# Clemapfel/kmer_index

Hardware: AMD Instinct MI355X
Metric: M queries/sec, DNA4 k=10 exact-match batch search, 1e8-bp text (higher is better)
Workload: dtype u32/u64

## Files before the change

include/kmx.h:

```cpp
#ifndef KMX_H
#define KMX_H

#include <stddef.h>
#include <stdint.h>

#ifdef __cplusplus
extern "C" {
#endif

#define KMX_VERSION 5
#define KMX_MAX_KS 32
#define KMX_MAX_DEVICES 16
#define KMX_QUERY_SIZE_RANGE 10000
#define KMX_SUBK_FANOUT_LIMIT 10000000ull

typedef enum kmx_status {
    KMX_OK = 0,
    KMX_ERR_INVALID_ARGUMENT = 1,
    KMX_ERR_HIP = 2,
    KMX_ERR_OUT_OF_MEMORY = 3,
    KMX_ERR_NO_DEVICE = 4,
    KMX_ERR_TOO_LARGE = 5
} kmx_status;

// ... 86 lines not shown
                                  const uint32_t** d_positions, const uint8_t** d_status);
kmx_status kmx_result_view(kmx_result* r, const uint64_t** hit_off, const uint32_t** positions,
                           const uint8_t** status, const uint8_t** kinds);

kmx_status kmx_result_parts(const kmx_result* r, uint32_t* n_parts);
kmx_status kmx_result_part_view_device(const kmx_result* r, uint32_t part, int32_t* device, uint64_t* q_begin, uint64_t* q_end,
                                       const uint64_t** d_hit_off, const uint32_t** d_positions, const uint8_t** d_status);
kmx_status kmx_index_devices(const kmx_index* index, uint32_t* n_devices, int32_t* devices);

kmx_status kmx_result_gather_device(kmx_result* r, int32_t dst_device, const uint64_t** d_hit_off, const uint32_t** d_positions,
                                    const uint8_t** d_status);

kmx_status kmx_result_masks(kmx_result* r, const uint64_t** mask_base, const uint64_t** mask_words,
                            const uint32_t** cand_count, const uint64_t** cand_src);
kmx_status kmx_index_arena_host(const kmx_index* index, const uint32_t** arena, uint64_t* n_elems);

kmx_status kmx_index_bucket_host(const kmx_index* index, uint32_t k, const uint8_t* ranks, const uint32_t** positions,
                                 uint32_t* count);

kmx_status kmx_index_levels(const kmx_index* index, uint32_t* levels);

#define KMX_PATH_INFO 1
typedef struct kmx_index_path_info {
    uint32_t struct_size;
    uint32_t fill_slots;
    uint32_t fill_nontemporal;
    uint32_t rec64;
    uint32_t tiny_cells;
    uint32_t scan_tile;
    uint32_t n_ks;
    uint32_t cell_shift[KMX_MAX_KS];
    uint32_t windows_tile;
} kmx_index_path_info;
kmx_status kmx_index_paths(const kmx_index* index, kmx_index_path_info* out);

typedef struct kmx_result_path_info {
    uint32_t struct_size;
    uint32_t small;
    uint32_t lookup_items;
    uint32_t lookup_pairs;
    uint32_t deferred_long;
    uint32_t tile_q_source;
    uint32_t spec_fill;
    uint32_t spec_ok;
    uint32_t fill_blocks;
    uint32_t fill_tiles;
    uint32_t prefix_plain;
    uint32_t prefix_small;
    uint32_t prefix_merge_small;
    uint32_t prefix_mid;
    uint32_t prefix_long;
    uint32_t prefix_large_chunks;
    uint64_t prefix_large_elems;
} kmx_result_path_info;
#define KMX_TILE_Q_NONE 0u
#define KMX_TILE_Q_PARTITION 1u
#define KMX_TILE_Q_SCAN 2u
kmx_status kmx_result_paths(const kmx_result* r, kmx_result_path_info* out);

void kmx_result_free(kmx_result* r);

#define KMX_APPROX_MAX_SUBST 3
#define KMX_APPROX_EDIT 1u
typedef struct kmx_approx_result kmx_approx_result;
kmx_status kmx_search_approx(const kmx_index* index, const uint8_t* qranks, const uint64_t* qoff, uint64_t nq,
                             uint32_t max_subst, uint32_t flags, kmx_approx_result** out);
kmx_status kmx_approx_counts(const kmx_approx_result* r, uint64_t* nq, uint64_t* n_hits, uint64_t* n_candidates,
                             uint32_t* n_chunks);
kmx_status kmx_approx_view(kmx_approx_result* r, const uint64_t** hit_off, const uint32_t** positions,
                           const uint8_t** mismatches, const uint8_t** status);
kmx_status kmx_approx_lengths(kmx_approx_result* r, const uint32_t** lengths);
void kmx_approx_free(kmx_approx_result* r);

#define KMX_APPROX_BOTH_STRANDS 1
kmx_status kmx_search_approx_strands(const kmx_index* index, const uint8_t* qranks, const uint64_t* qoff, uint64_t nq,
                                     uint32_t max_subst, uint32_t flags, const uint8_t* complement,
                                     kmx_approx_result** out);
kmx_status kmx_approx_strands(kmx_approx_result* r, const uint8_t** strands);

#define KMX_APPROX_REPORT 1
#define KMX_APPROX_LOCI 2u
#define KMX_APPROX_BEST 4u
typedef struct kmx_approx_options {
    uint32_t struct_size;
    uint32_t max_subst;
    uint32_t flags;
    uint32_t max_hits;
    const uint8_t* complement;
} kmx_approx_options;
kmx_status kmx_search_approx_opts(const kmx_index* index, const uint8_t* qranks, const uint64_t* qoff, uint64_t nq,
                                  const kmx_approx_options* options, kmx_approx_result** out);
kmx_status kmx_approx_found(kmx_approx_result* r, const uint64_t** found );

#define KMX_SEARCH_WINDOWS 1
typedef struct kmx_window_options {
    uint32_t struct_size;
    uint32_t w;
    uint32_t stride;
    uint32_t flags;
} kmx_window_options;
kmx_status kmx_search_windows(const kmx_index* index, const uint8_t* ranks, const uint64_t* roff, uint64_t nr,
                              const kmx_window_options* options, kmx_result** out);
kmx_status kmx_search_windows_device(const kmx_index* index, const void* d_ranks, const void* d_roff, uint64_t nr,
                                     const kmx_window_options* options, void* stream, kmx_result** inout);
kmx_status kmx_result_window_offsets(kmx_result* r, const uint64_t** win_off, const uint64_t** d_win_off, uint64_t* nr);

// ... 359 lines not shown
```

kmer_index_amd/build.py:

```python
import os
import shutil
import subprocess

HERE = os.path.dirname(os.path.abspath(__file__))
CSRC = os.path.join(HERE, "csrc")
LIB = os.path.join(HERE, "libkmx.so")
SOURCES = ["kmx_kernels.hip", "kmx_capi.hip", "kmx_build_sort.hip", "kmx_approx.hip", "kmx_vote.hip", "kmx_align.hip", "kmx_script.hip", "kmx_strands.hip", "kmx_pairs.hip", "kmx_rescue.hip", "kmx_tags.hip", "kmx_contigs.hip", "kmx_secondary.hip", "kmx_clip.hip", "kmx_supplementary.hip", "kmx_realign.hip", "kmx_pileup.hip", "kmx_host.cpp"]
HEADERS = ["kmx_types.h", "kmx_host.h", "kmx_kernels.h", "kmx_approx.h", "kmx_handle.h", "kmx_vote.h", "kmx_strands.h", "kmx_clips.h", "kmx_align_core.h", "kmx_script_core.h", "kmx_runs.h", "kmx_fold_core.h", os.path.join("..", "..", "include", "kmx.h")]


def _stale() -> bool:
    if not os.path.exists(LIB):
        return True
    t = os.path.getmtime(LIB)
    return any(os.path.getmtime(os.path.join(CSRC, f)) > t for f in SOURCES + HEADERS)


def build(force: bool = False, fill_e: int | None = None, verbose: bool = False, checked: bool = False) -> str:
    if not force and not _stale():
        return LIB
    hipcc = shutil.which("hipcc") or "/opt/rocm/bin/hipcc"
    cmd = [hipcc, "--offload-arch=gfx950", "-O3", "-std=c++17", "-fPIC", "-shared", "-pthread",
           "-Wall", "-Wno-unused-result", "-x", "hip"]
    if fill_e:
        cmd.append(f"-DKMX_FILL_E={fill_e}")
    for knob in ("KMX_PSORT_MULTIWAY_RUNS", "KMX_LOOKUP_OCC", "KMX_PSB_CPT", "KMX_PMERGE_MIN_AVG", "KMX_PMERGE_REG_RUNS", "KMX_PMERGE_REG_LEN", "KMX_PSORT_BAND_MIN", "KMX_SPLIT_TILE", "KMX_SPLIT_SCATTER_THREADS", "KMX_SPLIT", "KMX_NT_QUAD_LOADS", "KMX_PLAIN_QUAD_STORES", "KMX_VWAVE_OCC", "KMX_BAND", "KMX_MID_THREADS", "KMX_MID_OCC"):
        if os.environ.get(knob):
            cmd.append(f"-D{knob}={int(os.environ[knob])}")
    if os.environ.get("KMX_PHASE_TIMING"):
        cmd.append("-DKMX_PHASE_TIMING=1")
    if checked or os.environ.get("KMX_CHECKED"):
        cmd.append("-DKMX_CHECKED=1")
    cmd += [os.path.join(CSRC, f) for f in SOURCES] + ["-o", LIB]
    res = subprocess.run(cmd, capture_output=True, text=True)
    if res.returncode != 0:
        raise RuntimeError("hipcc failed:\n" + res.stdout + res.stderr)
    if verbose and (res.stdout or res.stderr):
        print(res.stdout + res.stderr)
    return LIB


if __name__ == "__main__":
    print(build(force=True, verbose=True))
```

kmer_index_amd/csrc/kmx_capi.hip:

```cpp
#include <hip/hip_runtime.h>

#include <algorithm>
#include <atomic>
#include <cstddef>
#include <cstdio>
#include <cstdlib>
#include <cstring>
#include <functional>
#include <memory>
#include <mutex>
#include <string>
#include <system_error>
#include <thread>
#include <utility>
#include <vector>

#include "kmx_approx.h"
#include "kmx_host.h"
#include "kmx_kernels.h"
#include "kmx_vote.h"

namespace {

thread_local std::string g_err;

kmx_status fail(kmx_status st, const std::string& msg)
{
    g_err = msg;
    return st;
}

#define HIP_TRY(expr)                                                                          \
    do {                                                                                       \
        hipError_t e__ = (expr);                                                               \
        if (e__ != hipSuccess) {                                                               \
            kmx_status st__ = (e__ == hipErrorOutOfMemory) ? KMX_ERR_OUT_OF_MEMORY : KMX_ERR_HIP; \
            if (e__ == hipErrorNoDevice || e__ == hipErrorInvalidDevice) st__ = KMX_ERR_NO_DEVICE; \
            return fail(st__, std::string(#expr) + ": " + hipGetErrorString(e__));             \
        }                                                                                      \
    } while (0)

#define KMX_TRY(expr) do { const kmx_status try_st__ = (expr); if (try_st__ != KMX_OK) return try_st__; } while (0)
struct DevBuf {
    void* p = nullptr;
    size_t cap = 0;
    hipError_t ensure(size_t bytes)
    {
        if (bytes <= cap) return hipSuccess;
        if (p) { (void)hipFree(p); p = nullptr; cap = 0; }
        size_t want = bytes + bytes / 16 + 256;
        hipError_t e = hipMalloc(&p, want);
        if (e != hipSuccess) { p = nullptr; return e; }
        cap = want;
        return hipSuccess;
    }
    void release()
    {
        if (p) (void)hipFree(p);
        p = nullptr; cap = 0;
    }
    template <typename T> T* as() const { return static_cast<T*>(p); }
};

struct HostBuf {
    void* p = nullptr;
    size_t cap = 0;
    bool pinned = false;
    bool ensure(size_t bytes)
    {
        if (bytes <= cap) return true;
        release();
// ... 62 lines not shown
    void drain()
    {
        for (auto& p : pending) {
            (void)hipEventSynchronize(p.b);
            float t = 0.f;
            if (hipEventElapsedTime(&t, p.a, p.b) == hipSuccess) { ms[p.id] += t; launches[p.id] += 1; }
            pool.push_back(p.a);
            pool.push_back(p.b);
        }
        pending.clear();
    }
    void destroy()
    {
        drain();
        for (auto e : pool) (void)hipEventDestroy(e);
        pool.clear();
    }
};

}

struct ResultPool {
    std::mutex mu;
    std::vector<kmx_result*> idle;
    std::vector<kmx_result*> pending;
    bool closed = false;
};
constexpr size_t kPoolMaxResults = 8;
constexpr size_t kPoolMaxBytes = size_t(256) << 20;
constexpr size_t kSmallView = size_t(256) << 10;

struct kmx_index {
    std::shared_ptr<ResultPool> pool = std::make_shared<ResultPool>();
    int device = 0;
    uint64_t n = 0;
    uint32_t sigma = 0;
    uint32_t range = KMX_QUERY_SIZE_RANGE;
    std::vector<uint32_t> ks;
    std::vector<uint32_t> table_kinds;
    std::vector<void*> allocs;
    uint64_t device_bytes = 0;
    uint64_t bytes_positions = 0, bytes_aligned = 0, bytes_cells = 0, bytes_levels = 0;
    KmxIndexDev* d_index = nullptr;
    KmxIndexDev* d_index_fast = nullptr;
    const KmxPlanEntry* d_plan_fast = nullptr;
    const uint32_t* d_arena = nullptr;
    unsigned long long* d_dbg = nullptr;
    struct ElemSizes { size_t n_offs, n_slots, n_ukeys, n_aoffs; };
    std::vector<ElemSizes> elem_sizes;
    std::vector<uint8_t> tail;
    KmxIndexDev h_header{};
    kmx::FillVariant fill_variant{12, true};
    bool rec32 = true;
    bool tiny_cells = false;
    bool broken = false;
    std::vector<uint32_t> host_arena;
    Stats stats;
    struct HostDir {
        std::once_flag once;
        kmx_status st = KMX_OK;
        std::string err;
        std::vector<uint32_t> offs;
        std::vector<uint64_t> ukeys;
    };
    std::unique_ptr<HostDir[]> host_dirs;
    std::vector<kmx_index*> peers;
    std::unique_ptr<kmx::PackedText> text = std::make_unique<kmx::PackedText>();
    kmx::ContigTable contigs;
    std::vector<uint64_t> h_contigs;
    size_t n_replicas() const { return 1 + peers.size(); }
    kmx_index* replica(size_t i) { return i ? peers[i - 1] : this; }
};

struct SearchCtx {
    kmx_index* ix = nullptr;
    const uint8_t* qr = nullptr;
    const uint64_t* qo = nullptr;
    hipStream_t s = nullptr;
    uint64_t tile_cap = 0, spec_tiles = 0;
    bool spec_fill = false;
    bool pending = false;
};

struct Tallies {
    uint64_t n_hits = 0, n_exact = 0, n_stitch = 0, n_prefix = 0, n_error = 0, n_none = 0, n_mask_words = 0;
    void reset() { *this = Tallies{}; }
    void operator+=(const Tallies& o) { n_hits += o.n_hits; n_exact += o.n_exact; n_stitch += o.n_stitch; n_prefix += o.n_prefix; n_error += o.n_error; n_none += o.n_none; n_mask_words += o.n_mask_words; }
    void derive_exact(uint64_t nq) { n_exact = nq - n_stitch - n_prefix - n_error - n_none; }
};
constexpr size_t kCtrBytes = KMX_CTR_COUNT * sizeof(unsigned long long);

struct kmx_result : Tallies {
    const kmx_index* index = nullptr;
    int device = 0;
    hipStream_t stream = nullptr;
    uint32_t flags = 0;
    uint64_t nq = 0;
    DevBuf src, cnt, c0, aux, key, p1, kind, status, stitch_list, prefix_list, short_list, hit_off, bsum, ctr, tile_q, out,
        mask_words, stitch_hits, plen, poff, ptmp, pitems, pbands, pcuts, pbanded, psplits, ptiles, pscnt, pscratch, pmid, in_qranks, in_qoff, win_cnt, win_off;
    unsigned long long* h_ctr = nullptr;
    HostBuf h_hit_off, h_positions, h_status, h_kinds, h_mask_base, h_mask_words, h_cand_count, h_cand_src, h_small;
    uint64_t* v_hit_off = nullptr; uint32_t* v_positions = nullptr; uint8_t* v_status = nullptr; uint8_t* v_kinds = nullptr;
    const uint64_t* m_base = nullptr; const uint64_t* m_words = nullptr; const uint32_t* m_ccnt = nullptr; const uint64_t* m_csrc = nullptr;
    uint32_t ctr_phase = 0;
    bool ctr_clean = false;
    HostBuf mailbox, small_in;
    DevBuf small_xchg;
    bool small_valid = false;
    bool host_valid = false, host_masks_valid = false;
    bool windows = false, h_win_valid = false;
    uint64_t win_nr = 0, win_n = 0;
    uint32_t win_w = 0, win_stride = 0;
    HostBuf h_win_off;
    bool last_had_stitch = false;
    bool last_had_long = false;
    bool last_had_pairs = false;
    struct PathRec { uint32_t small = 0, items = 0, pairs = 0, defer_long = 0, tile_q_source = 0, spec_fill = 0, spec_ok = 0, fill_blocks = 0, fill_tiles = 0;
                     uint32_t p_plain = 0, p_small = 0, p_merge = 0, p_mid = 0, p_long = 0, p_chunks = 0; uint64_t p_elems = 0; };
    PathRec path;
    std::shared_ptr<ResultPool> pool;
    SearchCtx ctx;
    hipEvent_t done = nullptr;
    bool quiesced = true;
    hipStream_t own_stream = nullptr;
    std::vector<kmx_result*> parts;
    std::vector<uint64_t> part_q0;
    std::vector<uint64_t> part_w0;
    bool chunked = false;
    bool host_chunk = false;
    kmx_result* worker = nullptr;
    kmx_result* worker2 = nullptr;
    DevBuf g_hit_off, g_out, g_status;
    int gather_device = -1;
    hipStream_t gather_stream = nullptr;

    Tallies& tally() { return *this; }
    template <typename R, typename F> static void each_device_buffer(R& r, F&& f)
    {
        for (auto* b : {&r.src, &r.cnt, &r.c0, &r.aux, &r.key, &r.p1, &r.kind, &r.status, &r.stitch_list, &r.prefix_list, &r.short_list, &r.hit_off, &r.bsum,
                        &r.ctr, &r.tile_q, &r.out, &r.mask_words, &r.stitch_hits, &r.plen, &r.poff, &r.ptmp, &r.pitems, &r.pbands, &r.pcuts, &r.pbanded, &r.psplits,
                        &r.ptiles, &r.pscnt, &r.pscratch, &r.pmid, &r.in_qranks, &r.in_qoff, &r.small_xchg, &r.win_cnt, &r.win_off})
            f(*b);
    }
    size_t device_bytes() const { size_t b = 0; each_device_buffer(*this, [&](const DevBuf& d) { b += d.cap; }); return b; }
    kmx::QueryDesc query_desc() const
    {
        return kmx::QueryDesc{src.as<uint64_t>(), cnt.as<uint32_t>(), c0.as<uint32_t>(), aux.as<uint64_t>(), key.as<uint64_t>(), p1.as<uint64_t>(),
                              kind.as<uint8_t>(), status.as<uint8_t>(), stitch_list.as<uint32_t>(), prefix_list.as<uint32_t>(), short_list.as<uint32_t>(), nullptr};
    }
    unsigned long long* ctr_block(uint32_t phase) const { return ctr.as<unsigned long long>() + phase * KMX_CTR_COUNT; }
    hipError_t ensure_h_ctr() { return h_ctr ? hipSuccess : hipHostMalloc(reinterpret_cast<void**>(&h_ctr), kCtrBytes, hipHostMallocDefault); }
    void view_own() { v_hit_off = h_hit_off.as<uint64_t>(); v_positions = h_positions.as<uint32_t>(); v_status = h_status.as<uint8_t>(); v_kinds = h_kinds.as<uint8_t>(); }
    void mask_view_own() { m_base = h_mask_base.as<uint64_t>(); m_words = h_mask_words.as<uint64_t>(); m_ccnt = h_cand_count.as<uint32_t>(); m_csrc = h_cand_src.as<uint64_t>(); }
    bool size_views(uint64_t pos_bytes)
    {
        const uint64_t nq1 = std::max<uint64_t>(nq, 1);
        const bool ok = h_hit_off.ensure((nq + 1) * 8) && h_status.ensure(nq1) && h_kinds.ensure(nq1) && h_positions.ensure(std::max<uint64_t>(pos_bytes, 4));
        if (ok) view_own();
        return ok;
    }
    bool size_mask_buffers()
    {
        const uint64_t nq1 = std::max<uint64_t>(nq, 1);
        return h_mask_base.ensure(nq1 * 8) && h_cand_count.ensure(nq1 * 4) && h_cand_src.ensure(nq1 * 8) &&
               h_mask_words.ensure(std::max<uint64_t>(n_mask_words, 1) * 8);
    }

    void release_gather()
    {
        (void)hipSetDevice(gather_device);
// ... 53 lines not shown
    launch();
    (void)hipEventRecord(b, s);
    ix->stats.pending.push_back({id, a, b});
}

template <typename T>
kmx_status upload(kmx_index* ix, const T* host, size_t count, const T** dev_out)
{
    void* p = nullptr;
    size_t bytes = std::max<size_t>(count * sizeof(T), 16) + 16;
    HIP_TRY(hipMalloc(&p, bytes));
    ix->allocs.push_back(p);
    ix->device_bytes += bytes;
    if (count) HIP_TRY(hipMemcpy(p, host, count * sizeof(T), hipMemcpyHostToDevice));
    *dev_out = static_cast<const T*>(p);
    return KMX_OK;
}

struct DeviceScratch {
    std::vector<void*> ptrs;
    ~DeviceScratch() { for (void* p : ptrs) (void)hipFree(p); }
    template <typename T> hipError_t get(T** out, size_t count)
    {
        void* p = nullptr;
        hipError_t e = hipMalloc(&p, count * sizeof(T) + 64);
        if (e == hipSuccess) { ptrs.push_back(p); *out = static_cast<T*>(p); }
        return e;
    }
};

kmx_status check_device()
{
    int count = 0;
    hipError_t e = hipGetDeviceCount(&count);
    if (e != hipSuccess || count <= 0)
        return fail(KMX_ERR_NO_DEVICE, "no HIP device visible: the kmx engine has no CPU search path");
    return KMX_OK;
}

}

static uint32_t cell_shift_for(uint32_t table_kind, uint64_t n_keys, uint64_t npos, uint64_t region, const kmx_options& o)
{
    if (table_kind != KMX_TABLE_DENSE || o.no_aligned_copy || region > npos) return 0;
    if (const char* e = getenv("KMX_CELLS")) { if (!atoi(e)) return 0; }
    const double c = double(npos) / double(n_keys);
    uint32_t shift = c <= 3.5 ? 3u : c <= 10.5 ? 4u : c <= 24.0 ? 5u : 0u;
    if (const char* e = getenv("KMX_CELL_SHIFT")) { const int v = atoi(e); if (v >= 3 && v <= 5) shift = uint32_t(v); }
    if (!shift) return 0;
    if ((n_keys << shift) > 8 * npos) return 0;
    return shift;
}
static inline uint64_t up32_elems(uint64_t v) { return (v + 31) & ~uint64_t(31); }

static hipError_t publish_headers(kmx_index* ix)
{
    hipError_t e = hipMemcpy(ix->d_index, &ix->h_header, sizeof(KmxIndexDev), hipMemcpyHostToDevice);
    if (e == hipSuccess && ix->d_index_fast) {
        KmxIndexDev hf = ix->h_header;
        if (ix->d_plan_fast) hf.plan = ix->d_plan_fast;
        e = hipMemcpy(ix->d_index_fast, &hf, sizeof hf, hipMemcpyHostToDevice);
    }
    return e;
}
static inline const KmxIndexDev* header_for(const kmx_index* ix, uint32_t flags)
{
    static const bool ref_plan_only = getenv("KMX_REFERENCE_PLAN") != nullptr;
    return ((flags & (KMX_SEARCH_KEEP_MASKS | KMX_SEARCH_REFERENCE_PLAN)) || !ix->d_index_fast || ref_plan_only) ? ix->d_index : ix->d_index_fast;
}

static kmx_status install_images_impl(std::vector<kmx::ElemImage>& images, const uint8_t* tail_kmax, uint64_t n, uint32_t sigma,
                                 uint32_t range, int device, const kmx_options& o, kmx_index** out, void* prebuilt_arena,
                                 uint64_t prebuilt_arena_elems = 0)
{
    auto* ix = new kmx_index();
    ix->device = device;
    ix->n = n;
    ix->sigma = sigma;
    ix->range = range;
    const uint32_t n_ks = uint32_t(images.size());
    uint32_t kmax = 0;
    for (auto& im : images) { ix->ks.push_back(im.k); kmax = std::max(kmax, im.k); }
    kmx_status st = KMX_OK;
    auto bail = [&](kmx_status s) { std::string keep = g_err; kmx_index_free(ix); g_err = keep; return s; };
    for (auto& im : images) {
        if (im.d_offs_prebuilt) ix->allocs.push_back(const_cast<uint32_t*>(im.d_offs_prebuilt));
        if (im.d_atab_prebuilt) ix->allocs.push_back(const_cast<uint32_t*>(im.d_atab_prebuilt));
        if (im.d_ukeys_prebuilt) ix->allocs.push_back(const_cast<uint64_t*>(im.d_ukeys_prebuilt));
        if (im.d_slots_prebuilt) ix->allocs.push_back(const_cast<KmxSlot*>(im.d_slots_prebuilt));
    }

    KmxIndexDev h{};
    h.n = n; h.sigma = sigma; h.n_ks = n_ks; h.kmax = kmax; h.range = range;
    for (uint32_t j = 0; j < 64; ++j) {
        unsigned __int128 v = 1;
        for (uint32_t t = 0; t < j; ++t) { v *= sigma; if (v > ~uint64_t(0)) { v = ~uint64_t(0); break; } }
        h.pw[j] = uint64_t(v);
    }
    uint64_t arena_elems = 0;
    for (auto& im : images) {
        if (!im.region) im.region = im.npos;
        if (im.region > im.npos) arena_elems = (arena_elems + 31) & ~uint64_t(31);
        arena_elems += im.region;
    }
    std::vector<uint32_t> cell_shift(n_ks, 0);
    std::vector<uint64_t> cell_base(n_ks, 0);
// ... 66 lines not shown
            ix->elem_sizes.back() = {size_t(nu + 1), size_t(cap), size_t(nu), size_t(0)};
        } else if (im.d_offs_prebuilt) {
            el.offs = im.d_offs_prebuilt;
            ix->device_bytes += (im.n_keys + 1) * 4;
            ix->elem_sizes.back().n_offs = im.n_keys + 1;
        } else if ((st = upload(ix, im.offs.data(), im.offs.size(), &el.offs)) != KMX_OK) return bail(st);
        if (im.d_atab_prebuilt) {
            el.atab = im.d_atab_prebuilt;
            ix->device_bytes += (im.n_keys + 1) * 4;
        } else if (im.table_kind == KMX_TABLE_DENSE && !im.atab.empty()) {
            if ((st = upload(ix, im.atab.data(), im.atab.size(), &el.atab)) != KMX_OK) return bail(st);
        }
        if (im.table_kind == KMX_TABLE_OPEN && !im.d_ukeys_prebuilt) {
            if ((st = upload(ix, im.slots.data(), im.slots.size(), &el.slots)) != KMX_OK) return bail(st);
            if ((st = upload(ix, im.ukeys.data(), im.ukeys.size(), &el.ukeys)) != KMX_OK) return bail(st);
        }
        el.dir = nullptr; el.dir_shift = 0; el.n_dir = 0;
        if (im.table_kind == KMX_TABLE_OPEN && el.n_ukeys >= 1024) {
            uint32_t key_bits = 1;
            while (key_bits < 64 && (im.n_keys - 1) >> key_bits) ++key_bits;
            uint32_t lg = 0;
            while ((uint64_t(1) << lg) < el.n_ukeys) ++lg;
            const uint32_t D = std::min<uint32_t>(std::min<uint32_t>(20, key_bits), lg > 8 ? lg - 4 : 4);
            void* p = nullptr;
            if (hipMalloc(&p, ((size_t(1) << D) + 1) * 4 + 64) == hipSuccess) {
                ix->allocs.push_back(p);
                ix->device_bytes += ((size_t(1) << D) + 1) * 4;
                el.dir = static_cast<const uint32_t*>(p);
                el.dir_shift = key_bits - D;
                el.n_dir = 1u << D;
                kmx::launch_build_dir(nullptr, el.ukeys, el.n_ukeys, el.dir_shift, el.n_dir, static_cast<uint32_t*>(p));
                hipError_t le = hipGetLastError();
                if (le == hipSuccess) le = hipDeviceSynchronize();
                if (le != hipSuccess) { fail(KMX_ERR_HIP, std::string("key directory: ") + hipGetErrorString(le)); return bail(KMX_ERR_HIP); }
            } else {
                (void)hipGetLastError();
            }
        }
        el.cnt8 = nullptr; el.cell_base = 0; el.cell_shift = 0; el.n_levels = 0;
        if (cell_shift[i]) {
            void* p = nullptr;
            hipError_t ce = hipMalloc(&p, im.n_keys + 64);
            if (ce == hipSuccess) {
                ix->allocs.push_back(p);
                ix->device_bytes += im.n_keys;
                (void)hipMemset(p, 0, im.n_keys + 64);
                kmx::launch_build_cells(nullptr, el.offs, h.arena + base, im.n_keys, cell_shift[i], const_cast<uint32_t*>(h.arena) + cell_base[i],
                                        static_cast<uint8_t*>(p));
                ce = hipGetLastError();
                if (ce == hipSuccess) ce = hipDeviceSynchronize();
            }
            if (ce != hipSuccess) { fail(ce == hipErrorOutOfMemory ? KMX_ERR_OUT_OF_MEMORY : KMX_ERR_HIP, std::string("cells: ") + hipGetErrorString(ce)); return bail(KMX_ERR_HIP); }
            el.cnt8 = static_cast<const uint8_t*>(p);
            if (im.npos <= 4 * im.n_keys) ix->tiny_cells = true;
            ix->bytes_cells += ((im.n_keys << cell_shift[i]) * 4) + im.n_keys;
            el.cell_base = cell_base[i];
            el.cell_shift = cell_shift[i];
            if (o.keep_host_arena) {
                ce = hipMemcpy(ix->host_arena.data() + cell_base[i], h.arena + cell_base[i], (im.n_keys << cell_shift[i]) * 4, hipMemcpyDeviceToHost);
                if (ce != hipSuccess) { fail(KMX_ERR_HIP, std::string("cells download: ") + hipGetErrorString(ce)); return bail(KMX_ERR_HIP); }
            }
        }
        base += im.region;
        im = kmx::ElemImage();
    }
    ix->host_dirs.reset(new kmx_index::HostDir[n_ks]);
    ix->tail.assign(tail_kmax, tail_kmax + kmax);
    if ((st = upload(ix, tail_kmax, kmax, &h.tail)) != KMX_OK) return bail(st);
    {
        std::vector<KmxPlanEntry> plan = kmx::make_plan_entries(ix->ks, range);
        if ((st = upload(ix, plan.data(), plan.size(), &h.plan)) != KMX_OK) return bail(st);
    }
    {
        const KmxIndexDev* d = nullptr;
        if ((st = upload(ix, &h, 1, &d)) != KMX_OK) return bail(st);
        ix->d_index = const_cast<KmxIndexDev*>(d);
        ix->h_header = h;
        std::vector<KmxPlanEntry> fast = kmx::make_fast_plan_entries(ix->ks, range, sigma);
        if ((st = upload(ix, fast.data(), fast.size(), &ix->d_plan_fast)) != KMX_OK) return bail(st);
        if ((st = upload(ix, &h, 1, &d)) != KMX_OK) return bail(st);
        ix->d_index_fast = const_cast<KmxIndexDev*>(d);
        const hipError_t pe = publish_headers(ix);
        if (pe != hipSuccess) { fail(KMX_ERR_HIP, std::string("header: ") + hipGetErrorString(pe)); return bail(KMX_ERR_HIP); }
    }
    *out = ix;
    return KMX_OK;
}

static kmx_status replicate_index(const kmx_index* src, int device, kmx_index** out)
{
    auto* ix = new kmx_index();
    ix->device = device;
    ix->n = src->n; ix->sigma = src->sigma; ix->range = src->range;
    ix->ks = src->ks; ix->table_kinds = src->table_kinds; ix->elem_sizes = src->elem_sizes; ix->tail = src->tail;
    ix->fill_variant = src->fill_variant; ix->rec32 = src->rec32; ix->tiny_cells = src->tiny_cells;
    ix->bytes_positions = src->bytes_positions; ix->bytes_aligned = src->bytes_aligned; ix->bytes_cells = src->bytes_cells; ix->bytes_levels = src->bytes_levels;
    auto bail = [&](kmx_status s) { std::string keep = g_err; kmx_index_free(ix); g_err = keep; return s; };
    hipError_t e = hipSetDevice(device);
    if (e != hipSuccess) { fail(KMX_ERR_NO_DEVICE, std::string("replica device: ") + hipGetErrorString(e)); return bail(KMX_ERR_NO_DEVICE); }
    kmx_status st = KMX_OK;
    auto clone = [&](const void* sp, size_t bytes, size_t pad, const void** dp) -> bool {
        *dp = nullptr;
        if (!sp) return true;
        void* p = nullptr;
        hipError_t e2 = hipMalloc(&p, std::max<size_t>(bytes, 16) + pad);
        if (e2 != hipSuccess) { st = fail(KMX_ERR_OUT_OF_MEMORY, std::string("replica: ") + hipGetErrorString(e2)); return false; }
        ix->allocs.push_back(p);
        ix->device_bytes += bytes;
        if (bytes) {
            e2 = hipMemcpyPeer(p, device, sp, src->device, bytes);
            if (e2 != hipSuccess) { st = fail(KMX_ERR_HIP, std::string("replica copy: ") + hipGetErrorString(e2)); return false; }
        }
        *dp = p;
        return true;
    };
    KmxIndexDev h = src->h_header;
    const void* p = nullptr;
    if (!clone(src->h_header.arena, h.arena_elems * 4 + KMX_ARENA_PAD, 0, &p)) return bail(st);
    h.arena = static_cast<const uint32_t*>(p); ix->d_arena = h.arena;
    if (!clone(src->h_header.tail, h.kmax, 16, &p)) return bail(st);
    h.tail = static_cast<const uint8_t*>(p);
    if (!clone(src->h_header.plan, size_t(h.range) * sizeof(KmxPlanEntry), 16, &p)) return bail(st);
    h.plan = static_cast<const KmxPlanEntry*>(p);
    if (!clone(src->d_plan_fast, src->d_plan_fast ? size_t(h.range) * sizeof(KmxPlanEntry) : 0, 16, &p)) return bail(st);
    ix->d_plan_fast = static_cast<const KmxPlanEntry*>(p);
    {
        void* d = nullptr;
        if (hipMalloc(&d, 16 * 8) == hipSuccess) { (void)hipMemset(d, 0, 16 * 8); ix->allocs.push_back(d); h.dbg = static_cast<unsigned long long*>(d); ix->d_dbg = h.dbg; }
        else { (void)hipGetLastError(); h.dbg = nullptr; }
    }
    for (uint32_t i = 0; i < h.n_ks; ++i) {
        const KmxElemDev& se = src->h_header.elems[i];
        KmxElemDev& de = h.elems[i];
        const auto& sz = src->elem_sizes[i];
        if (!clone(se.offs, sz.n_offs * 4, 16, &p)) return bail(st);
        de.offs = static_cast<const uint32_t*>(p);
        if (!clone(se.atab, sz.n_aoffs * 4, 16, &p)) return bail(st);
        de.atab = static_cast<const uint32_t*>(p);
        if (!clone(se.slots, sz.n_slots * sizeof(KmxSlot), 16, &p)) return bail(st);
        de.slots = static_cast<const KmxSlot*>(p);
        if (!clone(se.ukeys, sz.n_ukeys * 8, 16, &p)) return bail(st);
        de.ukeys = static_cast<const uint64_t*>(p);
        if (!clone(se.dir, se.dir ? (size_t(se.n_dir) + 1) * 4 : 0, 64, &p)) return bail(st);
        de.dir = static_cast<const uint32_t*>(p);
        if (!clone(se.cnt8, se.cnt8 ? size_t(se.n_keys) : 0, 64, &p)) return bail(st);
        de.cnt8 = static_cast<const uint8_t*>(p);
    }
    if (!clone(nullptr, 0, 0, &p)) return bail(st);
// ... 688 lines not shown
            if (he == hipSuccess && !hd.ukeys.empty()) he = hipMemcpy(hd.ukeys.data(), el.ukeys, hd.ukeys.size() * 8, hipMemcpyDeviceToHost);
            if (he != hipSuccess) { hd.st = KMX_ERR_HIP; hd.err = std::string("kmx_index_bucket_host: table download: ") + hipGetErrorString(he); }
        }
        if (have) (void)hipSetDevice(cur);
    });
    if (hd.st != KMX_OK) return fail(hd.st, hd.err);
    uint64_t g = h;
    if (el.table_kind == KMX_TABLE_OPEN) {
        const auto it = std::lower_bound(hd.ukeys.begin(), hd.ukeys.end(), h);
        if (it == hd.ukeys.end() || *it != h) return KMX_OK;
        g = uint64_t(it - hd.ukeys.begin());
    }
    if (g + 1 >= hd.offs.size()) return KMX_OK;
    const uint32_t a = hd.offs[g], b = hd.offs[g + 1];
    if (b == a) return KMX_OK;
    *positions = ix->host_arena.data() + el.arena_base + a;
    *count = b - a;
    return KMX_OK;
}

kmx_status kmx_index_levels(const kmx_index* ix, uint32_t* levels)
{
    if (!ix || !levels) return fail(KMX_ERR_INVALID_ARGUMENT, "kmx_index_levels: NULL argument");
    for (size_t i = 0; i < ix->ks.size(); ++i) levels[i] = ix->h_header.elems[i].n_levels;
    return KMX_OK;
}

kmx_status kmx_index_paths(const kmx_index* ix, kmx_index_path_info* out)
{
    if (!ix || !out || out->struct_size < sizeof(uint32_t)) return fail(KMX_ERR_INVALID_ARGUMENT, "kmx_index_paths: NULL argument or no struct_size");
    const kmx::FillVariant fv = kmx::effective_fill_variant(ix->fill_variant, ix->rec32);
    kmx_index_path_info v{};
    v.fill_slots = uint32_t(fv.e); v.fill_nontemporal = fv.nt; v.rec64 = !ix->rec32; v.tiny_cells = ix->tiny_cells;
    v.scan_tile = uint32_t(kmx::scan_tile());
    v.n_ks = uint32_t(ix->ks.size());
    for (size_t i = 0; i < ix->ks.size(); ++i) v.cell_shift[i] = ix->h_header.elems[i].cnt8 ? ix->h_header.elems[i].cell_shift : 0u;
    v.windows_tile = uint32_t(kmx::windows_tile());
    v.struct_size = std::min<uint32_t>(out->struct_size, uint32_t(sizeof v));
    memcpy(out, &v, v.struct_size);
    return KMX_OK;
}

kmx_status kmx_result_paths(const kmx_result* r, kmx_result_path_info* out)
{
    if (!r || !out || out->struct_size < sizeof(uint32_t)) return fail(KMX_ERR_INVALID_ARGUMENT, "kmx_result_paths: NULL argument or no struct_size");
    if (!r->parts.empty()) return fail(KMX_ERR_INVALID_ARGUMENT, "kmx_result_paths: a result of several parts has no single search to report");
    KMX_TRY(search_finish(const_cast<kmx_result*>(r)));
    kmx_result_path_info v{};
    v.small = r->path.small; v.lookup_items = r->path.items; v.lookup_pairs = r->path.pairs; v.deferred_long = r->path.defer_long;
    v.tile_q_source = r->path.tile_q_source; v.spec_fill = r->path.spec_fill; v.spec_ok = r->path.spec_ok;
    v.fill_blocks = r->path.fill_blocks; v.fill_tiles = r->path.fill_tiles;
    v.prefix_plain = r->path.p_plain; v.prefix_small = r->path.p_small; v.prefix_merge_small = r->path.p_merge; v.prefix_mid = r->path.p_mid;
    v.prefix_long = r->path.p_long; v.prefix_large_chunks = r->path.p_chunks; v.prefix_large_elems = r->path.p_elems;
    v.struct_size = std::min<uint32_t>(out->struct_size, uint32_t(sizeof v));
    memcpy(out, &v, v.struct_size);
    return KMX_OK;
}

kmx_status kmx_debug_words(const kmx_index* ix, uint64_t* words16)
{
    if (!ix || !words16 || !ix->d_dbg) return fail(KMX_ERR_INVALID_ARGUMENT, "kmx_debug_words: NULL argument");
    HIP_TRY(hipSetDevice(ix->device));
    HIP_TRY(hipDeviceSynchronize());
    HIP_TRY(hipMemcpy(words16, ix->d_dbg, 16 * 8, hipMemcpyDeviceToHost));
    return KMX_OK;
}

kmx_status kmx_stats_enable(kmx_index* ix, int enable)
{
    if (!ix) return fail(KMX_ERR_INVALID_ARGUMENT, "kmx_stats_enable: index is NULL");
    for (kmx_index* peer : ix->peers) (void)kmx_stats_enable(peer, enable);
    std::lock_guard<std::mutex> lock(ix->stats.mu);
    ix->stats.enabled = enable != 0;
    return KMX_OK;
}

kmx_status kmx_stats_get(kmx_index* ix, kmx_kernel_stat* stats, uint32_t* n)
{
    if (!ix || !stats || !n) return fail(KMX_ERR_INVALID_ARGUMENT, "kmx_stats_get: NULL argument");
    {
        std::lock_guard<std::mutex> lock(ix->stats.mu);
        (void)hipSetDevice(ix->device);
        ix->stats.drain();
        for (int i = 0; i < K_COUNT; ++i) stats[i] = kmx_kernel_stat{kKernelNames[i], ix->stats.launches[i], ix->stats.ms[i]};
    }
    for (kmx_index* peer : ix->peers) {
        std::lock_guard<std::mutex> lock(peer->stats.mu);
        (void)hipSetDevice(peer->device);
        peer->stats.drain();
        for (int i = 0; i < K_COUNT; ++i) { stats[i].launches += peer->stats.launches[i]; stats[i].total_ms += peer->stats.ms[i]; }
    }
    if (!ix->peers.empty()) (void)hipSetDevice(ix->device);
    *n = K_COUNT;
    return KMX_OK;
}

kmx_status kmx_stats_reset(kmx_index* ix)
{
    if (!ix) return fail(KMX_ERR_INVALID_ARGUMENT, "kmx_stats_reset: index is NULL");
    for (kmx_index* peer : ix->peers) (void)kmx_stats_reset(peer);
    std::lock_guard<std::mutex> lock(ix->stats.mu);
    (void)hipSetDevice(ix->device);
    ix->stats.drain();
    for (int i = 0; i < K_COUNT; ++i) { ix->stats.launches[i] = 0; ix->stats.ms[i] = 0; }
    return KMX_OK;
}

static kmx_status search_device_begin(const kmx_index* cix, const void* d_first, bool nonempty, kmx_result** inout, const char* fn, const char* what,
                                      kmx_index** ix_out)
{
    const std::string f = std::string(fn) + ": ";
    kmx_index* ix = const_cast<kmx_index*>(cix);
    if (ix->broken) return fail(KMX_ERR_HIP, "the index is unusable: a failed kmx_index_extend_query_size_range left its replicas inconsistent");
    if (!ix->peers.empty() && nonempty) {
        hipPointerAttribute_t attr{};
        if (hipPointerGetAttributes(&attr, d_first) != hipSuccess) { (void)hipGetLastError(); return fail(KMX_ERR_INVALID_ARGUMENT, f + what + " is not a device pointer"); }
        kmx_index* pick = nullptr;
        for (size_t i = 0; i < ix->n_replicas() && !pick; ++i)
            if (ix->replica(i)->device == attr.device) pick = ix->replica(i);
        if (!pick) return fail(KMX_ERR_INVALID_ARGUMENT, f + "the queries live on a device that holds no replica of this index");
        ix = pick;
    }
    HIP_TRY(hipSetDevice(ix->device));
    kmx_result* r = *inout;
    if (r && !r->parts.empty()) return fail(KMX_ERR_INVALID_ARGUMENT, f + "the result handle belongs to a multi-device search");
    if (r && r->device != ix->device && r->device_bytes())
        return fail(KMX_ERR_INVALID_ARGUMENT, f + "the result handle holds buffers on another device");
    if (!r) { r = take_result(ix); *inout = r; }
    else KMX_TRY(search_finish(r));
    *ix_out = ix;
    return KMX_OK;
}

static bool scan_hits(kmx_index* ix, kmx_result* r, hipStream_t s, uint64_t tile, uint64_t tile_cap, int items, const kmx::CounterPub& pub)
{
    bool published = false;
    timed(ix, K_SCAN, s, [&] {
        published = kmx::launch_scan_tiles(s, r->cnt.as<uint32_t>(), r->nq, r->bsum.as<uint64_t>(), r->hit_off.as<uint64_t>(),
                                           r->ctr_block(r->ctr_phase) + KMX_CTR_TOTAL_HITS, tile, tile_cap >= 2 ? tile_cap - 1 : 0,
                                           tile_cap >= 2 ? r->tile_q.as<uint32_t>() : nullptr, items, pub);
    });
    return published;
}

using LookupStep = std::function<int(const kmx::QueryDesc&, unsigned long long*, const KmxIndexDev*)>;
static kmx_status search_device_run(kmx_index* ix, kmx_result* r, const uint8_t* qr, const uint64_t* qo, uint64_t nq, uint32_t flags, hipStream_t s,
                                    const LookupStep& lookup)
{
    r->index = ix; r->device = ix->device; r->stream = s;
    (void)hipGetLastError();
    r->flags = flags;
    r->nq = nq;
    r->tally().reset();
    r->host_valid = r->host_masks_valid = false;
    r->small_valid = false;
    r->path = kmx_result::PathRec{};
    r->quiesced = false;
    HIP_TRY(r->ensure_h_ctr());
    HIP_TRY(r->hit_off.ensure((nq + 1) * 8));
    if (nq == 0) {
        HIP_TRY(hipMemsetAsync(r->hit_off.p, 0, 8, s));
        return KMX_OK;
    }
    const std::pair<DevBuf*, size_t> per_query[] = {{&r->src, 8}, {&r->cnt, 4}, {&r->c0, 4}, {&r->aux, 8}, {&r->key, 8}, {&r->p1, 8}, {&r->kind, 1},
                                                    {&r->status, 1}, {&r->stitch_list, 4}, {&r->prefix_list, 4}, {&r->short_list, 4}};
    for (const auto& b : per_query) HIP_TRY(b.first->ensure(nq * b.second));
    HIP_TRY(r->bsum.ensure(std::max(kmx::scan_blocks(nq), kmx::lookup_blocks(nq, 4)) * 8));
    if (r->ctr.cap < 2 * kCtrBytes) {
        HIP_TRY(r->ctr.ensure(2 * kCtrBytes));
        HIP_TRY(hipMemsetAsync(r->ctr.p, 0, 2 * kCtrBytes, s));
        r->ctr_phase = 0;
        r->ctr_clean = true;
    }
    const kmx::QueryDesc d = r->query_desc();
    if (!r->ctr_clean) {
        HIP_TRY(hipMemsetAsync(r->ctr.p, 0, 2 * kCtrBytes, s));
        r->ctr_clean = true;
    }
    r->ctr_phase ^= 1u;
    auto* ctr = r->ctr_block(r->ctr_phase);
    auto* ctr_next = r->ctr_block(r->ctr_phase ^ 1u);
    const KmxIndexDev* dix = header_for(ix, flags);

    const int items = lookup(d, ctr, dix);
    const kmx::FillVariant fv = kmx::effective_fill_variant(ix->fill_variant, ix->rec32);
    const uint64_t tile = kmx::fill_tile(fv);
    const uint64_t tile_cap = r->tile_q.cap / 4;
    const bool published = scan_hits(ix, r, s, tile, tile_cap, items, kmx::CounterPub{ctr, ctr_next, r->h_ctr});
    r->ctr_clean = published;
    const uint64_t spec_tiles = std::min<uint64_t>(tile_cap >= 2 ? tile_cap - 1 : 0, (r->out.cap / 4) / tile);
    const bool spec_fill = !(flags & KMX_SEARCH_COUNT_ONLY) && !r->last_had_stitch && spec_tiles > 0 && spec_tiles < 0x7FFFFFFFull;
    if (spec_fill)
        timed(ix, K_FILL, s, [&] {
            kmx::launch_fill(s, fv, ix->rec32, dix, ix->d_arena, r->hit_off.as<uint64_t>(), r->tile_q.as<uint32_t>(),
                             ctr + KMX_CTR_TOTAL_HITS, spec_tiles, d, r->out.as<uint32_t>());
        });
    r->path.spec_fill = spec_fill;
    if (!published) HIP_TRY(hipMemcpyAsync(r->h_ctr, ctr, kCtrBytes, hipMemcpyDeviceToHost, s));
    r->ctx = SearchCtx{ix, qr, qo, s, tile_cap, spec_tiles, spec_fill, true};
    if (flags & KMX_SEARCH_ASYNC) {
        if (!r->done) HIP_TRY(hipEventCreateWithFlags(&r->done, hipEventDisableTiming));
        HIP_TRY(hipEventRecord(r->done, s));
        r->pool = ix->pool;
        std::lock_guard<std::mutex> lock(ix->pool->mu);
        ix->pool->pending.push_back(r);
        return KMX_OK;
    }
    return search_finish(r);
}

kmx_status kmx_search_batch_device(const kmx_index* cix, const void* d_qranks, const void* d_qoff, uint64_t nq,
                                   uint32_t flags, void* stream, kmx_result** inout)
{
    if (!cix || !inout) return fail(KMX_ERR_INVALID_ARGUMENT, "kmx_search_batch_device: NULL argument");
    if (nq && (!d_qranks || !d_qoff)) return fail(KMX_ERR_INVALID_ARGUMENT, "kmx_search_batch_device: NULL query buffers");
    if (nq >= 0xFFFFFFFFull) return fail(KMX_ERR_INVALID_ARGUMENT, "kmx_search_batch_device: at most 2^32-2 queries per batch");
    kmx_index* ix = nullptr;
    KMX_TRY(search_device_begin(cix, d_qranks, nq != 0, inout, "kmx_search_batch_device", "d_qranks", &ix));
    hipStream_t s = static_cast<hipStream_t>(stream);
    const uint8_t* qr = static_cast<const uint8_t*>(d_qranks);
    const uint64_t* qo = static_cast<const uint64_t*>(d_qoff);
    kmx_result* r = *inout;
    r->windows = false;
    return search_device_run(ix, r, qr, qo, nq, flags, s, [&](const kmx::QueryDesc& d, unsigned long long* ctr, const KmxIndexDev* dix) {
        static const int force_items = getenv("KMX_LOOKUP_ITEMS") ? atoi(getenv("KMX_LOOKUP_ITEMS")) : 0;
        const bool pairs = force_items ? force_items == -4 : r->last_had_pairs;
        const int items = force_items ? (force_items == 8 ? 8 : 4) : (!pairs && ix->tiny_cells) ? 8 : 4;
        const bool defer_long = r->last_had_long;
        const uint32_t lflags = (flags & ~KMX_SEARCH_INTERNAL_DEFER_LONG) | (defer_long ? KMX_SEARCH_INTERNAL_DEFER_LONG : 0u);
        r->path.items = uint32_t(items); r->path.pairs = pairs; r->path.defer_long = defer_long;
        timed(ix, K_LOOKUP, s, [&] {
            kmx::launch_lookup(s, items, pairs, dix, qr, qo, nq, d, ctr, r->bsum.as<uint64_t>(), lflags);
            if (defer_long) kmx::launch_lookup_long(s, dix, qr, qo, nq, d, ctr, flags);
        });
        return items;
    });
}


static kmx_status windows_check(const char* fn, const kmx_index* ix, const kmx_window_options* o, const void* out, uint32_t* elem)
{
    const std::string f = std::string(fn) + ": ";
    if (!ix || !o || !out) return fail(KMX_ERR_INVALID_ARGUMENT, f + "NULL argument");
    if (o->struct_size < sizeof(kmx_window_options)) return fail(KMX_ERR_INVALID_ARGUMENT, f + "options->struct_size is too small");
    if (o->stride == 0) return fail(KMX_ERR_INVALID_ARGUMENT, f + "stride must be at least 1");
    if (o->flags & ~uint32_t(KMX_SEARCH_COUNT_ONLY))
        return fail(KMX_ERR_INVALID_ARGUMENT, f + "flags other than KMX_SEARCH_COUNT_ONLY have nothing to act on");
    for (size_t i = 0; i < ix->ks.size(); ++i)
        if (ix->ks[i] == o->w) { *elem = uint32_t(i); return KMX_OK; }
    return fail(KMX_ERR_INVALID_ARGUMENT, f + "w = " + std::to_string(o->w) + " is not the k of an element of the index");
}

static uint64_t window_count(uint64_t len, uint32_t w, uint32_t stride) { return len < w ? 0 : (len - w) / stride + 1; }

static kmx_status windows_device(const kmx_index* cix, const void* d_ranks, const void* d_roff, uint64_t nr, const kmx_window_options* o, uint32_t elem,
                                 hipStream_t s, kmx_result** inout, const uint64_t* known_nq, const char* fn)
{
    kmx_index* ix = nullptr;
    KMX_TRY(search_device_begin(cix, d_ranks ? d_ranks : d_roff, nr != 0, inout, fn, "d_ranks", &ix));
    kmx_result* r = *inout;
    const uint8_t* rk = static_cast<const uint8_t*>(d_ranks);
    const uint64_t* ro = static_cast<const uint64_t*>(d_roff);
    (void)hipGetLastError();
    r->windows = true;
    r->win_nr = nr;
    r->win_w = o->w; r->win_stride = o->stride; r->win_n = ix->n;
    r->h_win_valid = false;
    HIP_TRY(r->win_off.ensure((nr + 1) * 8));
    uint64_t nq = 0;
    if (nr == 0) {
        HIP_TRY(hipMemsetAsync(r->win_off.p, 0, 8, s));
    } else {
        HIP_TRY(r->win_cnt.ensure(nr * 4));
        HIP_TRY(r->bsum.ensure(kmx::scan_blocks(nr) * 8));
        HIP_TRY(r->ensure_h_ctr());
        timed(ix, K_SCAN, s, [&] {
            kmx::launch_window_counts(s, ro, nr, o->w, o->stride, r->win_cnt.as<uint32_t>());
            kmx::launch_scan(s, r->win_cnt.as<uint32_t>(), nr, r->bsum.as<uint64_t>(), r->win_off.as<uint64_t>(),
                             r->win_off.as<unsigned long long>() + nr);
        });
        if (known_nq) {
            nq = *known_nq;
        } else {
            HIP_TRY(hipMemcpyAsync(r->h_ctr, r->win_off.as<uint64_t>() + nr, 8, hipMemcpyDeviceToHost, s));
            HIP_TRY(hipStreamSynchronize(s));
            nq = r->h_ctr[0];
// ... 90 lines not shown
    if (!r->windows || !r->parts.empty())
        return fail(KMX_ERR_INVALID_ARGUMENT, "kmx_result_window_offsets: the result is not one of kmx_search_windows / kmx_search_windows_device");
    if (win_off) {
        if (!r->h_win_valid) {
            if (!r->h_win_off.ensure((r->win_nr + 1) * 8)) return fail(KMX_ERR_OUT_OF_MEMORY, "kmx_result_window_offsets: host allocation failed");
            HIP_TRY(hipSetDevice(r->device));
            HIP_TRY(hipMemcpyAsync(r->h_win_off.p, r->win_off.p, (r->win_nr + 1) * 8, hipMemcpyDeviceToHost, r->stream));
            HIP_TRY(hipStreamSynchronize(r->stream));
            r->h_win_valid = true;
        }
        *win_off = r->h_win_off.as<uint64_t>();
    }
    if (d_win_off) *d_win_off = r->win_off.as<uint64_t>();
    if (nr) *nr = r->win_nr;
    return KMX_OK;
}

struct BatchCounts {
    uint64_t stitch_groups, stitch_tiny, stitch_short, stitch_pending, stitch_more;
    uint64_t prefix_small, prefix_big, prefix_merge, prefix_mid, prefix_plain;
    uint64_t prefix_elems, max_runs;
    uint64_t total_hits, mask_words;
};

static kmx_status wait_counters(kmx_result* r)
{
    if (r->flags & KMX_SEARCH_ASYNC) {
        ResultPool& pool = *r->ctx.ix->pool;
        std::lock_guard<std::mutex> lock(pool.mu);
        pool.pending.erase(std::remove(pool.pending.begin(), pool.pending.end(), r), pool.pending.end());
    }
    HIP_TRY(hipSetDevice(r->device));
    if (r->done && (r->flags & KMX_SEARCH_ASYNC)) HIP_TRY(hipEventSynchronize(r->done));
    else HIP_TRY(hipStreamSynchronize(r->ctx.s));
    return KMX_OK;
}

static BatchCounts read_counts(kmx_result* r)
{
    const unsigned long long* h = r->h_ctr;
    BatchCounts c{};
    c.stitch_groups = h[KMX_CTR_STITCH]; c.stitch_tiny = h[KMX_CTR_STITCH_TINY]; c.stitch_short = h[KMX_CTR_STITCH_SHORT];
    c.stitch_pending = c.stitch_groups + c.stitch_tiny + c.stitch_short; c.stitch_more = h[KMX_CTR_STITCH_MORE];
    c.prefix_small = h[KMX_CTR_PREFIX]; c.prefix_big = h[KMX_CTR_PREFIX_BIG]; c.prefix_merge = h[KMX_CTR_PREFIX_MERGE];
    c.prefix_mid = h[KMX_CTR_PREFIX_MID]; c.prefix_plain = h[KMX_CTR_PREFIX_PLAIN]; c.prefix_elems = h[KMX_CTR_PREFIX_ELEMS]; c.max_runs = h[KMX_CTR_MAX_RUNS];
    c.total_hits = h[KMX_CTR_TOTAL_HITS]; c.mask_words = h[KMX_CTR_MASK_WORDS];
    r->n_stitch = c.stitch_pending + h[KMX_CTR_STITCH_RESOLVED];
    r->n_prefix = c.prefix_small + c.prefix_big + c.prefix_plain;
    r->n_error = h[KMX_CTR_ERROR]; r->n_none = h[KMX_CTR_NONE]; r->n_mask_words = c.mask_words;
    r->derive_exact(r->nq);
    r->last_had_stitch = c.stitch_pending != 0;
    r->last_had_long = h[KMX_CTR_LONG] != 0;
    r->last_had_pairs = r->n_stitch != 0;
    r->path.p_plain = uint32_t(c.prefix_plain); r->path.p_merge = uint32_t(c.prefix_merge); r->path.p_mid = uint32_t(c.prefix_mid);
    r->path.p_small = uint32_t(c.prefix_small - std::min(c.prefix_small, c.prefix_merge));
    r->path.p_long = uint32_t(c.prefix_big - std::min(c.prefix_big, c.prefix_mid));
    r->path.p_chunks = uint32_t(c.prefix_elems ? c.max_runs : 0); r->path.p_elems = c.prefix_elems;
    return c;
}

struct PrefixBigSizes {
    bool large, split_ok, bands_possible;
    uint64_t n_long, max_tiles, cap_items, cap_bands, cap_cuts;
    kmx::PrefixSplitRoom room;
};
static PrefixBigSizes prefix_big_sizes(const BatchCounts& c)
{
    static const bool no_bands = getenv("KMX_NO_BANDS") != nullptr;
    static const bool no_split = getenv("KMX_NO_SPLIT") != nullptr || no_bands;
    PrefixBigSizes z{};
    const uint64_t np = c.prefix_big, elems = c.prefix_elems;
    z.large = c.max_runs > 1 && elems > 0;
    z.max_tiles = z.large ? elems / kmx::prefix_merge_tile() + np : 0;
    z.n_long = np > c.prefix_mid ? np - c.prefix_mid : 0;
    z.split_ok = z.large && !no_split;
    const uint64_t n_large_max = elems / KMX_PSORT_BLOCK_CAP + 1;
    if (z.split_ok) {
        z.room.cap_splits = n_large_max; z.room.cap_tiles = elems / kmx::prefix_split_tile() + n_large_max;
        z.room.cap_counters = 3 * (elems / kmx::prefix_split_target() + n_large_max); z.room.cap_scratch = elems + 4 * n_large_max;
    }
    z.cap_items = z.n_long ? z.n_long + elems / KMX_PSORT_BLOCK_CAP + (z.split_ok ? elems / kmx::prefix_split_target() + n_large_max : 0) : 0;
    const bool chunks_banded = kmx::prefix_band_min() < KMX_PSORT_BLOCK_CAP;
    z.bands_possible = !no_bands && z.n_long && (z.large || chunks_banded);
    z.cap_bands = !z.bands_possible ? 0
                  : chunks_banded   ? z.n_long * (KMX_PSORT_BLOCK_CAP / kmx::prefix_band_target() + 1) + elems / kmx::prefix_band_target()
                                    : elems / kmx::prefix_band_target() + n_large_max;
    z.cap_cuts = std::min<uint64_t>((z.cap_bands + (chunks_banded ? z.n_long : n_large_max)) * kmx::prefix_band_runs(), uint64_t(1) << 26);
    return z;
}

struct Finish {
    kmx_result* r; kmx_index* ix; hipStream_t s;
    kmx::QueryDesc d;
    unsigned long long* ctr; const KmxIndexDev* dix; kmx::FillVariant fv; uint64_t tile;
    BatchCounts c;
    const uint64_t* hit_off() const { return r->hit_off.as<uint64_t>(); }
    uint32_t* out() const { return r->out.as<uint32_t>(); }
    kmx_status validate_stitch()
    {
        HIP_TRY(r->mask_words.ensure(c.mask_words * 8));
        static const bool no_survivors = getenv("KMX_NO_STITCH_HITS") != nullptr;
        if ((!(r->flags & KMX_SEARCH_COUNT_ONLY) || c.stitch_more) && !no_survivors && r->stitch_hits.ensure(c.mask_words * 64 * 4) == hipSuccess)
            d.stitch_hits = r->stitch_hits.as<uint32_t>();
        else
            (void)hipGetLastError();
        timed(ix, K_VALIDATE, s, [&] {
// ... 64 lines not shown
                    HIP_TRY(hipMemsetAsync(sr.counters, 0, sr.cap_counters * 4, s));
                } else {
                    (void)hipGetLastError();
                    sr = kmx::PrefixSplitRoom{};
                }
            }
            if (!z.bands_possible && !sr.splits) HIP_TRY(hipMemsetAsync(r->pbanded.p, 0, np * 4, s));
            else {
                timed(ix, K_PREFIX_BANDS, s, [&] {
                    kmx::launch_prefix_bands(s, dix, qo, d_big, np, hit_off(), ix->d_arena, r->pbanded.as<uint32_t>(), r->pbands.p, z.cap_bands,
                                             r->pcuts.as<uint32_t>(), z.cap_cuts, ctr + KMX_CTR_PSB_BANDS, sr);
                });
                if (sr.splits)
                    timed(ix, K_PREFIX_SPLIT, s, [&] {
                        kmx::launch_prefix_split(s, sr, ctr + KMX_CTR_PSB_BANDS, ix->d_arena, r->pbanded.as<uint32_t>(), ix->h_header.n, r->pitems.p, z.cap_items,
                                                 ctr + KMX_CTR_PSB_OTHER);
                    });
            }
        }
        if (z.large) {
            HIP_TRY(r->plen.ensure(np * 4));
            HIP_TRY(r->poff.ensure((np + 1) * 8));
            HIP_TRY(r->ptmp.ensure(z.max_tiles * T * 4));
            HIP_TRY(r->bsum.ensure(std::max(kmx::scan_blocks(np), kmx::scan_blocks(r->nq)) * 8));
            timed(ix, K_PREFIX_LEN, s, [&] { kmx::launch_prefix_len(s, d_big, np, r->pbanded.as<uint32_t>(), r->plen.as<uint32_t>()); });
            timed(ix, K_SCAN, s, [&] {
                kmx::launch_scan(s, r->plen.as<uint32_t>(), np, r->bsum.as<uint64_t>(), r->poff.as<uint64_t>(), ctr + KMX_CTR_PREFIX_TOTAL);
            });
        }
        if (n_mid) HIP_TRY(r->pmid.ensure(np * kmx::prefix_item_bytes()));
        timed(ix, K_PREFIX_SORT_BLOCK, s, [&] {
            kmx::launch_prefix_sort_block(s, dix, qo, d_big, np, n_mid, hit_off(), ix->d_arena, out(), z.large ? r->poff.as<uint64_t>() : nullptr,
                                          z.large ? r->ptmp.as<uint32_t>() : nullptr, r->pitems.p, z.cap_items, ctr + KMX_CTR_PSB_MERGE,
                                          r->pbanded.as<uint32_t>(), r->pbands.p, z.cap_bands, r->pcuts.as<uint32_t>(), ctr + KMX_CTR_PSB_BANDS, sr.scratch, r->pmid.p, ix->h_header.n, ix->d_dbg);
        });
        if (z.large) {
            uint32_t passes = 0;
            while ((uint64_t(1) << passes) < c.max_runs) ++passes;
            for (uint32_t p = 0; p < passes; ++p)
                timed(ix, K_MERGE_PASS, s, [&] {
                    kmx::launch_prefix_merge_pass(s, d_big, np, r->poff.as<uint64_t>(), z.max_tiles, hit_off(), out(), r->ptmp.as<uint32_t>(), p);
                });
        }
        return KMX_OK;
    }
};

static kmx_status search_finish(kmx_result* r)
{
    if (!r->ctx.pending) return KMX_OK;
    r->ctx.pending = false;
    KMX_TRY(wait_counters(r));
    kmx_index* ix = r->ctx.ix;
    const kmx::FillVariant fv = kmx::effective_fill_variant(ix->fill_variant, ix->rec32);
    Finish f{r, ix, r->ctx.s, r->query_desc(), r->ctr_block(r->ctr_phase), header_for(ix, r->flags), fv, kmx::fill_tile(fv), read_counts(r)};
    if (f.c.stitch_pending) KMX_TRY(f.validate_stitch());
    r->n_hits = f.c.total_hits;
    if (r->flags & KMX_SEARCH_COUNT_ONLY) return KMX_OK;
    if (r->n_hits == 0) {
        r->path.spec_ok = r->ctx.spec_fill; r->path.fill_blocks = uint32_t(r->ctx.spec_fill ? r->ctx.spec_tiles : 0);
        return KMX_OK;
    }
    KMX_TRY(f.fill_hits());
    if (f.c.stitch_pending && !f.d.stitch_hits) f.compact_stitch();
    f.prefix_small();
    if (f.c.prefix_big) KMX_TRY(f.prefix_big());
    HIP_TRY(hipGetLastError());
    return KMX_OK;
}

static kmx_status try_small(kmx_index* ix, kmx_result* r, const uint8_t* qranks, const uint64_t* qoff, uint64_t q0, uint64_t q1, uint32_t flags, bool* served)
{
    *served = false;
    const uint64_t nq = q1 - q0;
    static const bool no_small = getenv("KMX_NO_SMALL") != nullptr;
    const uint32_t n_sb = uint32_t((nq + KMX_SMALL_NQ - 1) / KMX_SMALL_NQ);
    bool small = nq && n_sb <= KMX_SMALL_BLOCKS && !(flags & KMX_SEARCH_COUNT_ONLY) && !no_small;
    KmxSmallArgs sargs{};
    for (uint32_t b = 0; small && b < n_sb; ++b) {
        const uint64_t b0 = q0 + uint64_t(b) * KMX_SMALL_NQ, b1 = std::min(q1, b0 + KMX_SMALL_NQ);
        const uint64_t letters = qoff[b1] - qoff[b0];
        small = (b1 - b0 + 1) * 8 + letters <= KMX_SMALL_IN_BYTES;
        sargs.nq[b] = uint16_t(b1 - b0);
        sargs.n_letters[b] = uint16_t(letters);
        uint32_t maybe_slow = 0;
        for (uint64_t i = b0; small && b1 - b0 > KMX_SMALL_WSLOW && i < b1; ++i)
            maybe_slow += std::find(ix->ks.begin(), ix->ks.end(), uint32_t(qoff[i + 1] - qoff[i])) == ix->ks.end();
        small = small && maybe_slow <= KMX_SMALL_WSLOW + KMX_SMALL_BSLOW;
    }
    const KmxSmallLayout L = kmx_small_layout(n_sb <= 1 ? 1u : n_sb <= 4 ? 4u : uint32_t(KMX_SMALL_BLOCKS));
    if (small && n_sb > 1 && r->small_xchg.ensure(KMX_SMALL_BLOCKS * 8) != hipSuccess) { (void)hipGetLastError(); small = false; }
    if (!small || !r->mailbox.ensure_pinned(L.bytes)) return KMX_OK;
    unsigned char* mb0 = r->mailbox.as<unsigned char>();
    KmxSmallHeader* hdrs = reinterpret_cast<KmxSmallHeader*>(mb0 + L.off_header);
    for (uint32_t b = 0; b < n_sb; ++b) {
        unsigned char* in = mb0 + size_t(b) * KMX_SMALL_IN_BYTES;
        const uint64_t b0 = q0 + uint64_t(b) * KMX_SMALL_NQ, lb = qoff[b0];
        uint64_t* in_off = reinterpret_cast<uint64_t*>(in);
        for (uint32_t i = 0; i <= sargs.nq[b]; ++i) in_off[i] = qoff[b0 + i] - lb;
        if (sargs.n_letters[b]) memcpy(in + (size_t(sargs.nq[b]) + 1) * 8, qranks + lb, sargs.n_letters[b]);
        hdrs[b].fallback = 2;
    }
    (void)hipGetLastError();
    unsigned long long* xchg = n_sb > 1 ? r->small_xchg.as<unsigned long long>() : nullptr;
    if (xchg) HIP_TRY(hipMemsetAsync(xchg, 0, KMX_SMALL_BLOCKS * 8, r->own_stream));
    timed(ix, K_SMALL, r->own_stream, [&] { kmx::launch_small(r->own_stream, header_for(ix, flags), ix->d_arena, mb0, L, n_sb, sargs, uint32_t(nq), xchg, flags); });
    HIP_TRY(hipGetLastError());
    HIP_TRY(hipStreamSynchronize(r->own_stream));
    for (uint32_t b = 0; b < n_sb; ++b)
        if (hdrs[b].fallback != 0) return KMX_OK;
    r->index = ix; r->device = ix->device; r->stream = r->own_stream; r->flags = flags & ~KMX_SEARCH_ASYNC; r->nq = nq;
    r->tally().reset();
    for (uint32_t b = 0; b < n_sb; ++b)
        r->tally() += Tallies{hdrs[b].n_hits, 0, hdrs[b].n_stitch, hdrs[b].n_prefix, hdrs[b].n_error, hdrs[b].n_none, hdrs[b].n_mask_words};
    r->derive_exact(nq);
    r->v_hit_off = reinterpret_cast<uint64_t*>(mb0 + L.off_hitoff); r->v_positions = reinterpret_cast<uint32_t*>(mb0 + L.off_pos);
    r->v_status = mb0 + L.off_status; r->v_kinds = mb0 + L.off_kinds;
    r->m_base = reinterpret_cast<const uint64_t*>(mb0 + L.off_mbase); r->m_words = reinterpret_cast<const uint64_t*>(mb0 + L.off_words);
    r->m_ccnt = reinterpret_cast<const uint32_t*>(mb0 + L.off_ccnt); r->m_csrc = reinterpret_cast<const uint64_t*>(mb0 + L.off_csrc);
    const uint64_t l0 = qoff[q0], n_letters = qoff[q1] - l0;
    if (!r->small_in.ensure_pageable((nq + 1) * 8 + n_letters + 16)) return fail(KMX_ERR_OUT_OF_MEMORY, "kmx_search_batch: host allocation failed");
    uint64_t* io = r->small_in.as<uint64_t>();
    for (uint64_t i = 0; i <= nq; ++i) io[i] = qoff[q0 + i] - l0;
    if (n_letters) memcpy(r->small_in.as<unsigned char>() + (nq + 1) * 8, qranks + l0, n_letters);
    r->host_valid = r->host_masks_valid = r->small_valid = r->quiesced = true;
    r->windows = false; r->path = kmx_result::PathRec{}; r->path.small = 1;
    r->last_had_stitch = r->last_had_pairs = r->last_had_long = false;
    r->pool = ix->pool;
    *served = true;
    return KMX_OK;
}

static kmx_status search_host_one(kmx_index* ix, const uint8_t* qranks, const uint64_t* qoff, uint64_t q0, uint64_t q1, uint32_t flags,
                                  kmx_result** inout, bool wait)
{
    KMX_TRY(host_handle(ix, inout, nullptr));
    kmx_result* r = *inout;
    bool served = false;
    KMX_TRY(try_small(ix, r, qranks, qoff, q0, q1, flags, &served));
    if (served) return KMX_OK;
    const uint64_t nq = q1 - q0;
    const uint64_t l0 = nq ? qoff[q0] : 0, n_letters = nq ? qoff[q1] - l0 : 0;
    if (l0 == 0) KMX_TRY(upload_queries(r, qranks, n_letters, qoff + q0, nq));
    else {
        std::vector<uint64_t> local(nq + 1);
        for (uint64_t i = 0; i <= nq; ++i) local[i] = qoff[q0 + i] - l0;
        KMX_TRY(upload_queries(r, qranks + l0, n_letters, local.data(), nq));
        HIP_TRY(hipStreamSynchronize(r->own_stream));
    }
    const uint32_t f = wait ? (flags & ~KMX_SEARCH_ASYNC) : (flags | KMX_SEARCH_ASYNC);
    KMX_TRY(kmx_search_batch_device(ix, r->in_qranks.p, r->in_qoff.p, nq, f, r->own_stream, inout));
    if (wait) {
        HIP_TRY(hipStreamSynchronize(r->own_stream));
        r->quiesced = true;
    }
    return KMX_OK;
}

static void append_part_host(kmx_result* parent, const kmx_result* p, uint64_t q0, uint64_t nqp, uint64_t h0, bool want_pos)
{
    memcpy(parent->v_hit_off + q0 + 1, p->v_hit_off + 1, nqp * 8);
    memcpy(parent->v_status + q0, p->v_status, nqp);
    memcpy(parent->v_kinds + q0, p->v_kinds, nqp);
    if (want_pos && p->n_hits) memcpy(parent->v_positions + h0, p->v_positions, p->n_hits * 4);
}
static hipError_t append_part_async(kmx_result* parent, const kmx_result* p, uint64_t q0, uint64_t nqp, uint64_t h0, bool want_pos)
{
    hipError_t e = hipSuccess;
    if (nqp) e = hipMemcpyAsync(parent->v_hit_off + q0 + 1, p->hit_off.as<uint64_t>() + 1, nqp * 8, hipMemcpyDeviceToHost, p->stream);
    if (e == hipSuccess && nqp) e = hipMemcpyAsync(parent->v_status + q0, p->status.p, nqp, hipMemcpyDeviceToHost, p->stream);
    if (e == hipSuccess && nqp) e = hipMemcpyAsync(parent->v_kinds + q0, p->kind.p, nqp, hipMemcpyDeviceToHost, p->stream);
    if (e == hipSuccess && want_pos && p->n_hits) e = hipMemcpyAsync(parent->v_positions + h0, p->out.p, p->n_hits * 4, hipMemcpyDeviceToHost, p->stream);
    return e;
}
static void rebase_part(kmx_result* parent, uint64_t q0, uint64_t q1, uint64_t h0)
{
    for (uint64_t q = q0 + 1; h0 && q <= q1; ++q) parent->v_hit_off[q] += h0;
}
struct CopyTask { std::thread th; kmx_status st = KMX_OK; std::string err; bool running = false; };
static kmx_status join_task(CopyTask& t)
// ... 760 lines not shown
```

kmer_index_amd/csrc/kmx_kernels.h:

```cpp
#pragma once
#include <hip/hip_runtime.h>
#include <stdint.h>
#include "kmx_types.h"


namespace kmx {

struct QueryDesc {
    uint64_t* src;
    uint32_t* cnt;
    uint32_t* c0;
    uint64_t* aux;
    uint64_t* key;
    uint64_t* p1;
    uint8_t* kind;
    uint8_t* status;
    uint32_t* stitch_list;
    uint32_t* prefix_list;
    uint32_t* short_list;
    uint32_t* stitch_hits;
};

uint64_t lookup_blocks(uint64_t nq, int items);
void launch_lookup(hipStream_t s, int items, bool pairs, const KmxIndexDev* ix, const uint8_t* qranks, const uint64_t* qoff,
                   uint64_t nq, const QueryDesc& d, unsigned long long* ctr, uint64_t* block_hits, uint32_t flags);
void launch_lookup_long(hipStream_t s, const KmxIndexDev* ix, const uint8_t* qranks, const uint64_t* qoff, uint64_t nq, const QueryDesc& d,
                        unsigned long long* ctr, uint32_t flags);
uint64_t windows_tile();
int windows_items();
void launch_window_counts(hipStream_t s, const uint64_t* roff, uint64_t nr, uint32_t w, uint32_t stride, uint32_t* cnt);
void launch_lookup_windows(hipStream_t s, const KmxIndexDev* ix, uint32_t elem, const uint8_t* ranks, const uint64_t* roff, const uint64_t* win_off,
                           uint64_t nr, uint64_t nq, uint32_t stride, const QueryDesc& d, unsigned long long* ctr, uint64_t* block_hits);
void launch_validate(hipStream_t s, const KmxIndexDev* ix, const uint32_t* arena, const uint8_t* qranks, const uint64_t* qoff,
                     const QueryDesc& d, uint64_t n_stitch, uint64_t n_more, uint64_t n_tiny, const uint32_t* tiny_list, uint64_t n_short,
                     uint64_t* mask_words, bool direct);
void launch_small(hipStream_t s, const KmxIndexDev* ix, const uint32_t* arena, unsigned char* mailbox, const KmxSmallLayout& layout, uint32_t n_blocks,
                  const KmxSmallArgs& args, uint32_t nq_total, unsigned long long* xchg, uint32_t flags);
uint64_t scan_blocks(uint64_t n);
void launch_build_dir(hipStream_t s, const uint64_t* d_ukeys, uint64_t n_ukeys, uint32_t shift, uint32_t n_dir, uint32_t* d_dir);
void launch_build_cells(hipStream_t s, const uint32_t* d_offs, const uint32_t* d_region, uint64_t n_keys, uint32_t cell_shift,
                        uint32_t* d_cells, uint8_t* d_cnt8);

struct SparseTables {
    uint64_t* d_ukeys = nullptr;
    uint32_t* d_offs = nullptr;
    KmxSlot* d_slots = nullptr;
    uint64_t n_ukeys = 0;
    uint32_t log2cap = 0;
};
hipError_t sort_kmer_positions(hipStream_t s, const uint8_t* d_text, uint64_t n, uint32_t k, uint32_t sigma, uint32_t key_bits,
                               uint32_t* d_positions);
hipError_t build_sparse_element(hipStream_t s, const uint8_t* d_text, uint64_t n, uint32_t k, uint32_t sigma, uint32_t key_bits,
                                uint32_t* d_positions, SparseTables* out);
hipError_t sort_pairs_u64(hipStream_t s, uint64_t* keys_a, uint32_t* vals_a, uint64_t* keys_b, uint32_t* vals_b, uint64_t n, uint32_t key_bits,
                          bool* in_b);
void launch_scan(hipStream_t s, const uint32_t* in, uint64_t n, uint64_t* bsum, uint64_t* out,
                 unsigned long long* total_out);
struct FillVariant {
    int e;
    bool nt;
};
struct CounterPub {
    const unsigned long long* cur = nullptr;
    unsigned long long* next = nullptr;
    unsigned long long* host = nullptr;
};
bool launch_scan_tiles(hipStream_t s, const uint32_t* in, uint64_t n, uint64_t* bsum, uint64_t* out,
                       unsigned long long* total_out, uint64_t tile, uint64_t n_tiles_cap, uint32_t* tile_q, int lookup_items,
                       const CounterPub& pub = CounterPub());
FillVariant effective_fill_variant(const FillVariant& v, bool rec32);
uint64_t scan_tile();
uint64_t fill_tile(const FillVariant& v);
void launch_partition(hipStream_t s, const uint64_t* off, uint64_t nq, uint64_t tile, uint64_t n_tiles, uint32_t* tile_q);
void launch_fill(hipStream_t s, const FillVariant& v, bool rec32, const KmxIndexDev* ix, const uint32_t* arena, const uint64_t* hit_off,
                 const uint32_t* tile_q, const unsigned long long* total_dev, uint64_t n_tiles, const QueryDesc& d, uint32_t* out);
void launch_compact(hipStream_t s, const uint32_t* arena, const QueryDesc& d, uint64_t n_stitch,
                    const uint64_t* mask_words, const uint64_t* hit_off, uint32_t* out);
void launch_prefix_len(hipStream_t s, const QueryDesc& d, uint64_t n_prefix, const uint32_t* banded, uint32_t* plen);
void launch_build_phase1(hipStream_t s, const uint8_t* d_text, uint64_t n, uint32_t k, uint32_t sigma, uint64_t n_keys,
                         uint32_t* d_hist, uint64_t* d_scratch_u64, uint64_t* d_bsum, uint32_t* d_offs, uint32_t* d_cursor,
// ... 42 lines not shown
```

kmer_index_amd/csrc/kmx_kernels.hip:

```cpp
#include <hip/hip_runtime.h>
#include <stdint.h>

#include <algorithm>
#include <atomic>
#include <type_traits>

#include "kmx_kernels.h"

#define KMX_BLOCK 256
#define KMX_WAVE 64
#define KMX_PSORT_PAIR_CAP 512
#ifndef KMX_PSORT_MULTIWAY_RUNS
#define KMX_PSORT_MULTIWAY_RUNS 4
#endif
#define KMX_PM_WAVE_EMAX (((KMX_PSORT_CAP + (KMX_WAVE - KMX_PSORT_MAX_RUNS / 2) - 1) / (KMX_WAVE - KMX_PSORT_MAX_RUNS / 2)) | 1)
#define KMX_PM_WAVE_PAD (KMX_PSORT_MAX_RUNS + KMX_PM_WAVE_EMAX + 5)
#define KMX_PM_TILE 4096
#define KMX_STAGE_CAP 1024
#define KMX_VGROUP 16
#define KMX_VGROUPS (KMX_WAVE / KMX_VGROUP)
#define KMX_VSLICES (64 / KMX_VGROUP)
#define KMX_VSTAGE (1024 / KMX_VGROUPS)
#define KMX_VCH 8

namespace kmx {

#define SRC_SLOW (uint64_t(1) << 63)
#define SRC_PREFIX (uint64_t(1) << 62)
#define SRC_FLAGS (SRC_SLOW | SRC_PREFIX)
#define KMX_P1_MORE (uint64_t(1) << 63)
#define KMX_P1_BIG (uint64_t(1) << 62)
#define KMX_P1_SWAP (uint64_t(1) << 61)
#define KMX_P1_DELTA_MASK 0x1FFFFFFFu
#define KMX_VBIG 1024
#define KMX_VWIDE_MIN 256
#define KMX_VWIDE 2048

__device__ __forceinline__ bool stitch_goes_big(uint32_t first_cnt, uint32_t filter_cnt)
{
    return first_cnt > KMX_VBIG && (filter_cnt > KMX_VWIDE || uint64_t(filter_cnt) * 8 < first_cnt);
}
__device__ __forceinline__ bool stitch_is_wide(uint64_t p1)
{
    return !(p1 & KMX_P1_BIG) && uint32_t(p1) > KMX_VWIDE_MIN && uint32_t(p1) <= KMX_VWIDE;
}
__device__ __forceinline__ uint32_t lane_id() { return threadIdx.x & (KMX_WAVE - 1); }

#define KMX_GLOBAL __attribute__((address_space(1)))
template <typename T>
__device__ __forceinline__ const KMX_GLOBAL T* as_global(const T* p)
{
    return (const KMX_GLOBAL T*)p;
}
#define KMX_LDS __attribute__((address_space(3)))
typedef unsigned long long u64x2 __attribute__((ext_vector_type(2)));
typedef uint32_t u32x4 __attribute__((ext_vector_type(4)));
typedef uint32_t u32x4_a4 __attribute__((ext_vector_type(4), aligned(4)));
#ifdef KMX_NT_QUAD_LOADS
#define KMX_LOAD_QUAD(p) __builtin_nontemporal_load(reinterpret_cast<const u32x4_a4*>(p))
// ... 323 lines not shown
                if (j == 0) {
                    extra = r; extra_delta = uint32_t(mm);
                    track = !(flags & KMX_SEARCH_KEEP_MASKS) && nparts > 1 && sparse_buckets(el) && r.cnt != 0 && r.cnt <= KMX_VRESOLVE;
                    if (track) {
                        alive = 0;
#pragma unroll
                        for (uint32_t i = 0; i < KMX_VRESOLVE; ++i) {
                            const uint32_t a = ar[r.src + (i < r.cnt ? i : 0u)];
                            cand[i] = a - uint32_t(mm);
                            alive |= uint32_t(i < r.cnt && a >= uint32_t(mm)) << i;
                        }
                    }
                } else if (track && r.cnt) {
                    follow(r, uint32_t(mm));
                }
                all = r.cnt != 0;
            }
            if (all && ranks_ok) {
                if (nparts == 1) { kind = KMX_KIND_EXACT; src = r.src; cnt = r.cnt; }
                else {
                    kind = KMX_KIND_STITCH; src = r.src; c0 = r.cnt;
                    key = extra.src;
                    p1 = (uint64_t(extra_delta) << 32) | extra.cnt | (nparts > 2 ? KMX_P1_MORE : 0);
                    if (!(flags & KMX_SEARCH_KEEP_MASKS) && stitch_goes_big(r.cnt, extra.cnt)) p1 |= KMX_P1_BIG;
                    if (track) {
                        uint32_t fmask = 0;
                        for (uint32_t t = 0; t < r.cnt; ++t) {
                            const uint32_t b = ar[r.src + t];
#pragma unroll
                            for (uint32_t i = 0; i < KMX_VRESOLVE; ++i) fmask |= uint32_t(((alive >> i) & 1u) && cand[i] == b) << t;
                        }
                        const uint32_t lo = fmask ? uint32_t(__ffs(int(fmask))) - 1u : 0u, len = uint32_t(__popc(fmask));
                        if ((fmask >> lo) == (1u << len) - 1u) {
                            resolved = true;
                            src = r.src + lo;
                            cnt = len;
                        }
                    }
                }
            }
        }
        if (!ranks_ok) { status = KMX_Q_BAD_RANK; kind = KMX_KIND_NONE; cnt = 0; }
    }
    o.src = src; o.aux = aux; o.key = key; o.p1 = p1; o.cnt = cnt; o.c0 = c0; o.kind = kind; o.status = status; o.resolved = resolved;
}

struct BlockCounters {
    unsigned int n_long, base_long;
    unsigned int n_stitch, n_stitch_tiny, n_stitch_short, n_resolved, n_prefix, n_prefix_big, n_prefix_merge, n_prefix_mid, n_prefix_plain, n_error, n_none, n_more;
    unsigned long long words, pelems, hits;
    unsigned int max_runs;
    unsigned int base_stitch, base_stitch_tiny, base_stitch_short, base_prefix, base_prefix_big;
    unsigned long long base_words;
    unsigned int max_fan_exp;
    unsigned int small_keys;
};

template <bool SMALL>
__device__ __forceinline__ bool hash16(const u32x4_a1& w, uint32_t len, uint32_t sigma, uint64_t& h)
{
    uint64_t lo = uint64_t(w[0]) | (uint64_t(w[1]) << 32), hi = uint64_t(w[2]) | (uint64_t(w[3]) << 32);
    {
        const uint32_t sh = (16u - len) * 8u;
        const uint32_t s6 = sh & 63u;
        const uint64_t carry = s6 ? lo >> (64u - s6) : 0;
        const uint64_t hi1 = (hi << s6) | carry, lo1 = lo << s6;
        hi = sh >= 128u ? 0 : sh >= 64u ? lo1 : hi1;
        lo = sh >= 64u ? 0 : lo1;
    }
    const uint32_t wd[4] = {uint32_t(lo), uint32_t(lo >> 32), uint32_t(hi), uint32_t(hi >> 32)};
    uint32_t top = 0;
    if (SMALL) {
        uint32_t acc = 0;
#pragma unroll
        for (uint32_t j = 0; j < 16; ++j) {
            const uint32_t r = (wd[j >> 2] >> (8 * (j & 3))) & 0xFFu;
            top = max(top, r);
            acc = __umul24(acc, sigma) + r;
        }
        h = acc;
    } else {
        uint64_t acc = 0;
#pragma unroll
        for (uint32_t j = 0; j < 16; ++j) {
            const uint32_t r = (wd[j >> 2] >> (8 * (j & 3))) & 0xFFu;
            top = max(top, r);
            acc = acc * sigma + r;
        }
        h = acc;
    }
    return top < sigma;
}
__device__ __forceinline__ const char* probe_first_addr(const KmxElemDev* el, uint64_t h)
{
    if (el->table_kind == KMX_TABLE_DENSE)
        return el->cnt8 ? reinterpret_cast<const char*>(el->cnt8 + (h & ~uint64_t(15)))
                        : reinterpret_cast<const char*>((el->atab ? el->atab : el->offs) + h);
    return reinterpret_cast<const char*>(el->slots + slot_hash_dev(h, el->log2cap));
}
__device__ __forceinline__ Run probe_finish(const KmxElemDev* el, uint64_t h, const u32x4_a1& pr)
{
    Run r{0, 0};
    if (el->table_kind == KMX_TABLE_DENSE) {
        if (el->cnt8) {
            const uint32_t b = uint32_t(h) & 15u;
            const uint32_t wsel = (b >> 2) == 0 ? pr[0] : (b >> 2) == 1 ? pr[1] : (b >> 2) == 2 ? pr[2] : pr[3];
            const uint32_t c = (wsel >> ((b & 3u) * 8u)) & 0xFFu;
            if (c != 255u) { r.src = el->cell_base + (h << el->cell_shift); r.cnt = c; }
            else {
                const KMX_GLOBAL uint32_t* offs = as_global(el->offs);
                const uint32_t a = offs[h], e = offs[h + 1];
                r.src = el->arena_base + a; r.cnt = e - a;
            }
        }
        else if (el->atab) { r.src = el->arena_base + (pr[0] & ~31u); r.cnt = atab_count(pr[0], pr[1]); }
        else { r.src = el->arena_base + pr[0]; r.cnt = pr[1] - pr[0]; }
        return r;
    }
    const KMX_GLOBAL KmxSlot* slots = as_global(el->slots);
    const uint64_t mask = (uint64_t(1) << el->log2cap) - 1;
    uint64_t s = slot_hash_dev(h, el->log2cap);
    uint64_t key = uint64_t(pr[0]) | (uint64_t(pr[1]) << 32);
    uint32_t off = pr[2], c = pr[3];
    while (c != 0 && key != h) {
        s = (s + 1) & mask;
        const u64x2 raw = *(const KMX_GLOBAL u64x2*)(slots + s);
        key = raw.x; off = uint32_t(raw.y); c = uint32_t(raw.y >> 32);
    }
    if (c) { r.src = el->arena_base + off; r.cnt = c; }
    return r;
}

#define KMX_PLAN_LDS 256

#ifndef KMX_LOOKUP_OCC
#define KMX_LOOKUP_OCC 4
#endif
template <int ITEMS, bool PAIRS>
__global__ __launch_bounds__(KMX_BLOCK, PAIRS ? KMX_LOOKUP_OCC : (ITEMS > 4 ? 4 : 5)) void k_lookup(const KmxIndexDev* __restrict__ ix,
                                                      const uint8_t* __restrict__ qranks,
                                                      const uint64_t* __restrict__ qoff, uint64_t nq,
                                                      QueryDesc d, unsigned long long* __restrict__ ctr,
                                                      uint64_t* __restrict__ block_hits, uint32_t flags)
{
    __shared__ BlockCounters bc;
    __shared__ KmxElemDev elems_s[KMX_MAX_KS];
    __shared__ uint32_t plan_s[KMX_PLAN_LDS];
    static_assert(KMX_PLAN_LDS == KMX_BLOCK, "one planner entry per thread");
    if (threadIdx.x == 0) {
        bc.n_long = 0;
        bc.n_stitch = bc.n_stitch_tiny = bc.n_stitch_short = bc.n_resolved = bc.n_prefix = bc.n_prefix_big = bc.n_prefix_merge = bc.n_prefix_mid = bc.n_prefix_plain = bc.n_error = bc.n_none = bc.n_more = 0;
        bc.words = bc.pelems = bc.hits = 0;
        bc.max_runs = 0;
        unsigned int j = 0;
        while (j < 63 && ix->pw[j + 1] <= KMX_SUBK_FANOUT_LIMIT) ++j;
        bc.max_fan_exp = j;
        unsigned int small = ix->sigma < (1u << 24) ? 1u : 0u;
        for (uint32_t e = 0; e < ix->n_ks; ++e) {
            const uint64_t nk = ix->elems[e].n_keys;
            if (nk > (uint64_t(1) << 32) || nk / ix->sigma > (uint64_t(1) << 24)) small = 0;
        }
        bc.small_keys = small;
    }
    {
        const uint32_t n_words = ix->n_ks * uint32_t(sizeof(KmxElemDev) / 8);
        const uint64_t* __restrict__ srcw = reinterpret_cast<const uint64_t*>(ix->elems);
        uint64_t* dstw = reinterpret_cast<uint64_t*>(elems_s);
        for (uint32_t i = threadIdx.x; i < n_words; i += KMX_BLOCK) dstw[i] = srcw[i];
        plan_s[threadIdx.x] = threadIdx.x < ix->range ? ((const KMX_GLOBAL uint32_t*)ix->plan)[threadIdx.x] : 0u;
    }
    const uint8_t* __restrict__ qend = qranks + qoff[nq];
    __syncthreads();

    uint8_t kinds[ITEMS];
    unsigned int locs[ITEMS];
    unsigned long long locw[ITEMS];
    bool done[ITEMS];
    uint64_t my_hits = 0;
    const uint32_t sigma = ix->sigma, range = ix->range;
    const bool small_keys = __builtin_amdgcn_readfirstlane(int(bc.small_keys)) != 0;
    const uint8_t* __restrict__ dummy = reinterpret_cast<const uint8_t*>(ix);

    unsigned int my_resolved = 0, my_err = 0, my_none = 0;
    auto emit = [&](int it, uint64_t q, uint8_t kind, uint8_t status, uint64_t src, uint64_t aux, uint64_t key, uint64_t p1, uint32_t cnt,
                    uint32_t c0, bool resolved) {
        unsigned int loc = 0;
        unsigned long long loc_words = 0;
        if (kind == KMX_KIND_STITCH && !resolved) {
            const uint32_t pc = uint32_t(p1);
            if (min(c0, pc) <= KMX_VTINY && max(c0, pc) <= 2 * KMX_VTINY) {
                loc = atomicAdd(&bc.n_stitch_tiny, 1u) | 0x80000000u;
            } else if (!(p1 & (KMX_P1_MORE | KMX_P1_BIG)) && min(c0, pc) <= KMX_VSHORT && max(c0, pc) <= KMX_VSTAGE) {
                loc = atomicAdd(&bc.n_stitch_short, 1u) | 0x40000000u;
                if (pc < c0) p1 |= KMX_P1_SWAP;
            } else {
                if ((p1 & (KMX_P1_MORE | KMX_P1_BIG)) || stitch_is_wide(p1)) atomicAdd(&bc.n_more, 1u);
                loc = atomicAdd(&bc.n_stitch, 1u);
            }
            loc_words = atomicAdd(&bc.words, (unsigned long long)(uint64_t(c0) / 64 + 1));
        }
        if (kind == KMX_KIND_PREFIX) {
            const uint32_t plen = cnt - uint32_t(__popcll(aux));
            if (c0 < 2 || plen < 2) {
                loc = 0xFFFFFFFFu;
                atomicAdd(&bc.n_prefix_plain, 1u);
            } else if (KMX_PSORT_IS_SMALL(c0, plen)) {
                loc = atomicAdd(&bc.n_prefix, 1u);
                if (KMX_PSORT_IS_MERGE(c0, plen)) atomicAdd(&bc.n_prefix_merge, 1u);
            } else {
                loc = atomicAdd(&bc.n_prefix_big, 1u) | 0x80000000u;
                if (plen <= KMX_PSORT_MID_CAP) atomicAdd(&bc.n_prefix_mid, 1u);
                if (plen > KMX_PSORT_BLOCK_CAP) {
                    atomicAdd(&bc.pelems, (unsigned long long)plen);
                    atomicMax(&bc.max_runs, (plen + KMX_PSORT_BLOCK_CAP - 1) / KMX_PSORT_BLOCK_CAP);
                }
            }
        }
        my_resolved += resolved;
        my_err += status != KMX_Q_OK;
        my_none += status == KMX_Q_OK && kind == KMX_KIND_NONE;
        kinds[it] = !resolved ? kind : uint8_t(KMX_KIND_NONE);
        locs[it] = loc;
        locw[it] = loc_words;
        my_hits += cnt;
        d.src[q] = (kind == KMX_KIND_STITCH && !resolved) ? (src | SRC_SLOW) : (kind == KMX_KIND_PREFIX ? (src | SRC_FLAGS) : src);
        d.cnt[q] = cnt;
        d.kind[q] = kind;
        d.status[q] = status;
        if (kind == KMX_KIND_STITCH) {
            if (!resolved) {
                d.c0[q] = c0;
                d.key[q] = key;
                d.p1[q] = p1;
            }
        } else if (kind == KMX_KIND_PREFIX) {
            d.c0[q] = c0;
            d.aux[q] = aux;
            d.key[q] = key;
        }
    };

    uint64_t qb[ITEMS];
    uint32_t qm[ITEMS];
    uint32_t praw[ITEMS];
#pragma unroll
    for (int it = 0; it < ITEMS; ++it) {
        const uint64_t q = (uint64_t(blockIdx.x) * ITEMS + it) * KMX_BLOCK + threadIdx.x;
        const uint64_t qq = q < nq ? q : nq - 1;
        qb[it] = qoff[qq];
        const uint64_t mlen = qoff[qq + 1] - qb[it];
        qm[it] = mlen > 0xFFFFFFFFull ? 0xFFFFFFFFu : uint32_t(mlen);
        kinds[it] = KMX_KIND_NONE;
        locs[it] = 0;
        locw[it] = 0;
    }
#pragma unroll
    for (int it = 0; it < ITEMS; ++it)
        praw[it] = plan_effective(((const KMX_GLOBAL uint32_t*)ix->plan)[min(qm[it], range - 1)]);

    {
        uint32_t eab[ITEMS];
        bool two[ITEMS];
        u32x4_a1 wa[ITEMS], wb[ITEMS];
        unsigned int n_none = 0, n_err = 0;
#pragma unroll
        for (int it = 0; it < ITEMS; ++it) {
            const uint64_t q = (uint64_t(blockIdx.x) * ITEMS + it) * KMX_BLOCK + threadIdx.x;
            const uint32_t m = qm[it], scheme = praw[it] & 0xFF, e = (praw[it] >> 8) & 0xFF;
            const uint32_t kb = elems_s[e].k;
            const bool live = q < nq && m > 0 && m < range;
            const bool one = live && scheme == KMX_SCHEME_SINGLE && kb == m && m <= 16 && qranks + qb[it] + 16 <= qend;
            bool t = false;
            uint32_t ea = e, off = 0;
            if (PAIRS && live && !one && m < KMX_PLAN_LDS) {
                if (scheme == KMX_SCHEME_SINGLE) {
                    const uint32_t rest = m < 2 * kb ? m - kb : 0u;
                    t = m > kb && m <= 2 * kb && kb <= 16 && (rest == 0 || kb - rest <= bc.max_fan_exp);
                    off = m - kb;
                } else if (scheme == KMX_SCHEME_MULTI && ((praw[it] >> 16) & KMX_PLAN_NPARTS_MASK) == 2 && m > kb) {
                    const uint32_t p2 = plan_s[m - kb];
                    ea = (p2 >> 8) & 0xFF;
                    const uint32_t ka = elems_s[ea].k;
                    t = (p2 & 0xFF) != KMX_SCHEME_NONE && ka + kb == m && ka <= 16 && kb <= 16;
                    off = m - kb;
                }
                t = t && qranks + qb[it] + off + 16 <= qend;
            }
            done[it] = one || t;
            two[it] = t;
            eab[it] = ea | (e << 8) | (off << 16);
            wa[it] = *reinterpret_cast<const u32x4_a1*>(done[it] ? qranks + qb[it] : dummy);
            if (PAIRS) wb[it] = *reinterpret_cast<const u32x4_a1*>(t ? qranks + qb[it] + off : dummy);
        }
        uint64_t ha[ITEMS], hb[ITEMS];
        bool oka[ITEMS], okb[ITEMS];
        u32x4_a1 pa[ITEMS], pb[ITEMS];
#pragma unroll
        for (int it = 0; it < ITEMS; ++it) {
            const KmxElemDev* ela = &elems_s[eab[it] & 0xFF];
            const KmxElemDev* elb = &elems_s[(eab[it] >> 8) & 0xFF];
            okb[it] = true; hb[it] = 0;
            if (small_keys) {
                oka[it] = hash16<true>(wa[it], done[it] ? ela->k : 0u, sigma, ha[it]);
                if (PAIRS) okb[it] = hash16<true>(wb[it], two[it] ? elb->k : 0u, sigma, hb[it]);
            } else {
                oka[it] = hash16<false>(wa[it], done[it] ? ela->k : 0u, sigma, ha[it]);
                if (PAIRS) okb[it] = hash16<false>(wb[it], two[it] ? elb->k : 0u, sigma, hb[it]);
            }
            pa[it] = *(const KMX_GLOBAL u32x4_a1*)((done[it] && oka[it]) ? probe_first_addr(ela, ha[it]) : reinterpret_cast<const char*>(dummy));
            if (PAIRS) pb[it] = *(const KMX_GLOBAL u32x4_a1*)((two[it] && okb[it]) ? probe_first_addr(elb, hb[it]) : reinterpret_cast<const char*>(dummy));
        }
        struct Pend {
            bool two, tiny, first_is_short;
            uint8_t kind, status;
            uint64_t src, key, p1;
            uint32_t c0, off, pc;
            u32x4 s0, s1, l0, l1, l2, l3;
        };
        const KMX_GLOBAL uint32_t* ar = as_global(ix->arena);
        auto stage1 = [&](int it) -> Pend {
            Pend P{};
            P.two = false; P.tiny = false; P.first_is_short = true; P.kind = KMX_KIND_NONE; P.status = KMX_Q_OK; P.src = P.key = P.p1 = 0; P.c0 = P.off = P.pc = 0;
            const uint64_t q = (uint64_t(blockIdx.x) * ITEMS + it) * KMX_BLOCK + threadIdx.x;
            Run ra{0, 0}, rb{0, 0};
            if (done[it]) {
                const KmxElemDev* ela = &elems_s[eab[it] & 0xFF];
                if (oka[it]) ra = probe_finish(ela, ha[it], pa[it]);
                if (!PAIRS || !two[it]) {
                    const uint8_t status = oka[it] ? KMX_Q_OK : KMX_Q_BAD_RANK;
                    n_err += status != KMX_Q_OK;
// ... 93 lines not shown
    for (int it = 0; it < ITEMS; ++it) {
        if (done[it]) continue;
        const uint64_t q = (uint64_t(blockIdx.x) * ITEMS + it) * KMX_BLOCK + threadIdx.x;
        if (q >= nq) continue;
        const uint64_t b = qoff[q];
        const uint64_t m = qoff[q + 1] - b;
        if (m > 0 && m < range) {
            const KmxPlanEntry pe = plan_unpack(plan_effective(m < KMX_PLAN_LDS ? plan_s[m] : ((const KMX_GLOBAL uint32_t*)ix->plan)[m]));
            if (pe.scheme == KMX_SCHEME_SINGLE) {
                const uint32_t k = elems_s[pe.elem].k;
                if (m > uint64_t(k) * KMX_LONG_PARTS) {
                    const unsigned int slot = atomicAdd(&bc.n_long, 1u);
                    if (flags & KMX_SEARCH_INTERNAL_DEFER_LONG) {
                        kinds[it] = 0xFF;
                        locs[it] = slot;
                        continue;
                    }
                }
            }
        }
        LookupOut lo;
        lookup_query(ix, elems_s, qranks + b, m, qend, flags & ~KMX_SEARCH_INTERNAL_DEFER_LONG, lo);
        emit(it, q, lo.kind, lo.status, lo.src, lo.aux, lo.key, lo.p1, lo.cnt, lo.c0, lo.resolved);
    }

    if (my_resolved) atomicAdd(&bc.n_resolved, my_resolved);
    if (my_err) atomicAdd(&bc.n_error, my_err);
    if (my_none) atomicAdd(&bc.n_none, my_none);
    for (int off = 32; off > 0; off >>= 1) my_hits += __shfl_xor(my_hits, off);
    if (lane_id() == 0 && my_hits) atomicAdd(&bc.hits, (unsigned long long)my_hits);
    __syncthreads();
    if (threadIdx.x == 0) {
        if (block_hits) block_hits[blockIdx.x] = bc.hits;
        if (bc.n_stitch | bc.n_stitch_tiny | bc.n_stitch_short) {
            if (bc.n_stitch) bc.base_stitch = (unsigned int)atomicAdd(&ctr[KMX_CTR_STITCH], (unsigned long long)bc.n_stitch);
            if (bc.n_stitch_tiny) bc.base_stitch_tiny = (unsigned int)atomicAdd(&ctr[KMX_CTR_STITCH_TINY], (unsigned long long)bc.n_stitch_tiny);
            if (bc.n_stitch_short) bc.base_stitch_short = (unsigned int)atomicAdd(&ctr[KMX_CTR_STITCH_SHORT], (unsigned long long)bc.n_stitch_short);
            bc.base_words = atomicAdd(&ctr[KMX_CTR_MASK_WORDS], bc.words);
            if (bc.n_more) atomicAdd(&ctr[KMX_CTR_STITCH_MORE], (unsigned long long)bc.n_more);
        }
        if (bc.n_prefix) bc.base_prefix = (unsigned int)atomicAdd(&ctr[KMX_CTR_PREFIX], (unsigned long long)bc.n_prefix);
        if (bc.n_prefix_merge) atomicAdd(&ctr[KMX_CTR_PREFIX_MERGE], (unsigned long long)bc.n_prefix_merge);
        if (bc.n_prefix_mid) atomicAdd(&ctr[KMX_CTR_PREFIX_MID], (unsigned long long)bc.n_prefix_mid);
        if (bc.n_prefix_plain) atomicAdd(&ctr[KMX_CTR_PREFIX_PLAIN], (unsigned long long)bc.n_prefix_plain);
        if (bc.n_prefix_big) {
            bc.base_prefix_big = (unsigned int)atomicAdd(&ctr[KMX_CTR_PREFIX_BIG], (unsigned long long)bc.n_prefix_big);
            if (bc.pelems) atomicAdd(&ctr[KMX_CTR_PREFIX_ELEMS], bc.pelems);
            if (bc.max_runs) atomicMax(&ctr[KMX_CTR_MAX_RUNS], (unsigned long long)bc.max_runs);
        }
        if (bc.n_long) bc.base_long = (unsigned int)atomicAdd(&ctr[KMX_CTR_LONG], (unsigned long long)bc.n_long);
        if (bc.n_resolved) atomicAdd(&ctr[KMX_CTR_STITCH_RESOLVED], (unsigned long long)bc.n_resolved);
        if (bc.n_error) atomicAdd(&ctr[KMX_CTR_ERROR], (unsigned long long)bc.n_error);
        if (bc.n_none) atomicAdd(&ctr[KMX_CTR_NONE], (unsigned long long)bc.n_none);
    }
    __syncthreads();
#pragma unroll
    for (int it = 0; it < ITEMS; ++it) {
        const uint64_t q = (uint64_t(blockIdx.x) * ITEMS + it) * KMX_BLOCK + threadIdx.x;
        if (kinds[it] == 0xFF) {
            d.short_list[nq - 1 - (bc.base_long + locs[it])] = uint32_t(q);
        } else if (kinds[it] == KMX_KIND_STITCH) {
            d.aux[q] = bc.base_words + locw[it];
            if (locs[it] & 0x80000000u) d.stitch_list[nq - 1 - (bc.base_stitch_tiny + (locs[it] & 0x3FFFFFFFu))] = uint32_t(q);
            else if (locs[it] & 0x40000000u) d.short_list[bc.base_stitch_short + (locs[it] & 0x3FFFFFFFu)] = uint32_t(q);
            else d.stitch_list[bc.base_stitch + locs[it]] = uint32_t(q);
        } else if (kinds[it] == KMX_KIND_PREFIX && locs[it] != 0xFFFFFFFFu) {
            if (locs[it] & 0x80000000u) d.prefix_list[nq - 1 - (bc.base_prefix_big + (locs[it] & 0x7FFFFFFFu))] = uint32_t(q);
            else d.prefix_list[bc.base_prefix + locs[it]] = uint32_t(q);
        }
    }
}

__global__ __launch_bounds__(KMX_BLOCK) void k_lookup_long(const KmxIndexDev* __restrict__ ix, const uint8_t* __restrict__ qranks,
                                                           const uint64_t* __restrict__ qoff, uint64_t nq, QueryDesc d,
                                                           unsigned long long* __restrict__ ctr, uint32_t flags)
{
    const uint32_t lane = lane_id();
    const uint64_t wave = (uint64_t(blockIdx.x) * KMX_BLOCK + threadIdx.x) / KMX_WAVE;
    const uint64_t n_waves = uint64_t(gridDim.x) * (KMX_BLOCK / KMX_WAVE);
    const uint64_t n_long = ctr[KMX_CTR_LONG];
    const uint8_t* __restrict__ qend = qranks + qoff[nq];
    const uint32_t sigma = ix->sigma;
    for (uint64_t i = wave; i < n_long; i += n_waves) {
        const uint32_t q = d.short_list[nq - 1 - i];
        const uint64_t b = qoff[q], m = qoff[q + 1] - b;
        const uint8_t* __restrict__ qr = qranks + b;
        const KmxPlanEntry pe = load_plan(ix, m);
        const KmxElemDev* __restrict__ el = &ix->elems[pe.elem];
        const uint32_t k = el->k;
        const uint32_t P = uint32_t(m / k), rest = uint32_t(m % k);
        const bool fan = rest && ix->pw[k - rest] > KMX_SUBK_FANOUT_LIMIT;
        const uint32_t n_parts = P + ((rest && !fan) ? 1u : 0u);
        uint32_t my_stop = 0xFFFFFFFFu;
        Run first{0, 0}, last{0, 0};
        for (uint32_t j = lane; j < n_parts; j += KMX_WAVE) {
            const uint64_t start = j < P ? uint64_t(j) * k : m - k;
            uint64_t h;
            const bool ok = rank_hash(qr + start, k, sigma, h, qend);
            Run r{0, 0};
            if (ok) r = probe(el, h);
            if ((!ok || r.cnt == 0) && my_stop == 0xFFFFFFFFu) my_stop = 2 * j + (ok ? 1u : 0u);
            if (j == 0) first = r;
            if (j == n_parts - 1) last = r;
        }
        uint32_t stop = my_stop;
        for (int off = 32; off > 0; off >>= 1) stop = min(stop, uint32_t(__shfl_xor(int(stop), off)));
// ... 160 lines not shown
    for (int i = 0; i < KMX_WIN_ITEMS; ++i) {
        const bool live = q0 + i < tile_end;
        status[i] = (live && !ok[i]) ? uint8_t(KMX_Q_BAD_RANK) : uint8_t(KMX_Q_OK);
        kind[i] = runs[i].cnt ? uint8_t(KMX_KIND_EXACT) : uint8_t(KMX_KIND_NONE);
        if (!runs[i].cnt) runs[i].src = 0;
        my_err += live && !ok[i];
        my_none += live && ok[i] && !runs[i].cnt;
        my_hits += runs[i].cnt;
    }
    if (q0 + KMX_WIN_ITEMS <= tile_end) {
#pragma unroll
        for (int i = 0; i < KMX_WIN_ITEMS; i += 2) {
            u64x2 v;
            v.x = runs[i].src; v.y = runs[i + 1].src;
            *reinterpret_cast<u64x2*>(d.src + q0 + i) = v;
        }
#pragma unroll
        for (int i = 0; i < KMX_WIN_ITEMS; i += 4) {
            u32x4 v;
            v.x = runs[i].cnt; v.y = runs[i + 1].cnt; v.z = runs[i + 2].cnt; v.w = runs[i + 3].cnt;
            *reinterpret_cast<u32x4*>(d.cnt + q0 + i) = v;
        }
        uint64_t kw = 0, sw = 0;
#pragma unroll
        for (int i = 0; i < KMX_WIN_ITEMS; ++i) { kw |= uint64_t(kind[i]) << (8 * i); sw |= uint64_t(status[i]) << (8 * i); }
        *reinterpret_cast<uint64_t*>(d.kind + q0) = kw;
        *reinterpret_cast<uint64_t*>(d.status + q0) = sw;
    } else {
#pragma unroll
        for (int i = 0; i < KMX_WIN_ITEMS; ++i) {
            if (q0 + i < tile_end) {
                d.src[q0 + i] = runs[i].src;
                d.cnt[q0 + i] = runs[i].cnt;
                d.kind[q0 + i] = kind[i];
                d.status[q0 + i] = status[i];
            }
        }
    }
    for (int off = 32; off > 0; off >>= 1) {
        my_hits += __shfl_xor(my_hits, off);
        my_err += __shfl_xor(my_err, off);
        my_none += __shfl_xor(my_none, off);
    }
    if (lane_id() == 0) {
        if (my_hits) atomicAdd(&s_hits, (unsigned long long)my_hits);
        if (my_err) atomicAdd(&s_err, my_err);
        if (my_none) atomicAdd(&s_none, my_none);
    }
    __syncthreads();
    if (threadIdx.x == 0) {
        block_hits[blockIdx.x] = s_hits;
        if (s_err) atomicAdd(&ctr[KMX_CTR_ERROR], (unsigned long long)s_err);
        if (s_none) atomicAdd(&ctr[KMX_CTR_NONE], (unsigned long long)s_none);
    }
}

__device__ __forceinline__ bool stitch_parts_hold(const KmxIndexDev* __restrict__ ix, const uint32_t* __restrict__ arena,
                                                  const uint8_t* __restrict__ qranks, const uint64_t* __restrict__ qoff,
                                                  uint32_t q, uint32_t p, uint32_t gl, uint32_t stride = KMX_VGROUP,
                                                  uint32_t skip_start = 0xFFFFFFFFu)
{
    const uint64_t b = qoff[q];
    const uint64_t m = qoff[q + 1] - b;
    const uint8_t* __restrict__ qr = qranks + b;
    const uint8_t* __restrict__ qend = qranks + qoff[q + 1];
    const uint32_t sigma = ix->sigma;
    const KmxPlanEntry pe = load_plan(ix, m);
    bool good = true;
    if (pe.scheme == KMX_SCHEME_SINGLE) {
        const KmxElemDev* __restrict__ el = &ix->elems[pe.elem];
        const uint32_t k = el->k;
        const uint32_t P = uint32_t(m / k);
        const uint32_t n_extra = P - 1 + ((m % k) ? 1 : 0);
        for (uint32_t e = gl; e < n_extra && good; e += stride) {
            const uint64_t start = (e < P - 1) ? uint64_t(e + 1) * k : (m - k);
            if (uint32_t(start) == skip_start) continue;
            uint64_t h;
            rank_hash(qr + start, k, sigma, h, qend);
            const Run r = probe(el, h);
            const uint32_t x = p + uint32_t(start);
            const uint64_t lb = lower_bound_dev<uint32_t>(arena + r.src, r.cnt, x);
            good = lb < r.cnt && arena[r.src + lb] == x;
        }
    } else {
        const uint32_t n_extra = pe.nparts - 1u;
        uint64_t mm = m;
        uint32_t walked = 0;
        for (uint32_t e = gl; e < n_extra && good; e += stride) {
            const KmxElemDev* __restrict__ el = nullptr;
            uint32_t k = 0;
            for (; walked <= e; ++walked) {
                const KmxPlanEntry en = load_plan_chain(ix, mm);
                el = &ix->elems[en.elem];
                k = el->k;
                mm -= k;
            }
            if (uint32_t(mm) == skip_start) continue;
            uint64_t h;
            rank_hash(qr + mm, k, sigma, h, qend);
            const Run r = probe(el, h);
            const uint32_t x = p + uint32_t(mm);
            const uint64_t lb = lower_bound_dev<uint32_t>(arena + r.src, r.cnt, x);
            good = lb < r.cnt && arena[r.src + lb] == x;
        }
    }
    return good;
// ... 2172 lines not shown
        if (tid == KMX_WAVE) cut[1] = c1;
    }
    __syncthreads();
    const uint32_t a0 = cut[0], a1 = cut[1], b0 = d0 - a0;
    const uint32_t nA = a1 - a0, nB = n_out - nA;
    for (uint32_t t = tid; t < n_out + 2; t += KMX_BLOCK) {
        uint32_t v = KMX_PM_SENT;
        if (t < nA) v = A[a0 + t];
        else if (t > nA && t < n_out + 1) v = B[b0 + (t - nA - 1)];
        buf[t] = v;
    }
    __syncthreads();
    const KMX_LDS uint32_t* lb = (const KMX_LDS uint32_t*)buf;
    const uint32_t dg = min(tid * E, n_out);
    const uint32_t lo = merge_path_cut(lb, nA, lb + (nA + 1), nB, dg);
    uint32_t x[E];
    merge_chunk<int(E), false>(lb + lo, lb + (nA + 1 + dg - lo), nullptr, nullptr, E, x);
    __syncthreads();
#pragma unroll
    for (uint32_t j = 0; j < E; ++j)
        if (dg + j < n_out) buf[dg + j] = x[j];
    __syncthreads();
    for (uint32_t t = tid; t < n_out; t += KMX_BLOCK) dst[o0 + t] = buf[t];
}

static void allow_big_lds(const void* fn, size_t bytes, int which)
{
    static std::atomic<uint64_t> done[3] = {{0}, {0}, {0}};
    int dev = 0;
    if (hipGetDevice(&dev) != hipSuccess) { (void)hipGetLastError(); return; }
    const uint64_t bit = uint64_t(1) << (dev & 63);
    if (done[which].load(std::memory_order_acquire) & bit) return;
    (void)hipFuncSetAttribute(fn, hipFuncAttributeMaxDynamicSharedMemorySize, int(bytes));
    done[which].fetch_or(bit, std::memory_order_release);
}

static inline unsigned int blocks_for(uint64_t n, uint64_t per_block)
{
    uint64_t b = (n + per_block - 1) / per_block;
    return (unsigned int)(b ? b : 1);
}

uint64_t lookup_blocks(uint64_t nq, int items) { return blocks_for(nq, uint64_t(KMX_BLOCK) * uint64_t(items)); }

void launch_lookup(hipStream_t s, int items, bool pairs, const KmxIndexDev* ix, const uint8_t* qranks, const uint64_t* qoff,
                   uint64_t nq, const QueryDesc& d, unsigned long long* ctr, uint64_t* block_hits, uint32_t flags)
{
    const dim3 grid(blocks_for(nq, uint64_t(KMX_BLOCK) * uint64_t(items))), block(KMX_BLOCK);
    if (pairs) hipLaunchKernelGGL((k_lookup<4, true>), grid, block, 0, s, ix, qranks, qoff, nq, d, ctr, block_hits, flags);
    else if (items == 8) hipLaunchKernelGGL((k_lookup<8, false>), grid, block, 0, s, ix, qranks, qoff, nq, d, ctr, block_hits, flags);
    else hipLaunchKernelGGL((k_lookup<4, false>), grid, block, 0, s, ix, qranks, qoff, nq, d, ctr, block_hits, flags);
}

uint64_t windows_tile() { return KMX_WIN_TILE; }
int windows_items() { return KMX_WIN_ITEMS; }

void launch_window_counts(hipStream_t s, const uint64_t* roff, uint64_t nr, uint32_t w, uint32_t stride, uint32_t* cnt)
{
    hipLaunchKernelGGL(k_window_counts, dim3(blocks_for(nr, KMX_BLOCK)), dim3(KMX_BLOCK), 0, s, roff, nr, w, stride, cnt);
}

void launch_lookup_windows(hipStream_t s, const KmxIndexDev* ix, uint32_t elem, const uint8_t* ranks, const uint64_t* roff, const uint64_t* win_off,
                           uint64_t nr, uint64_t nq, uint32_t stride, const QueryDesc& d, unsigned long long* ctr, uint64_t* block_hits)
{
    static_assert(KMX_WIN_ITEMS == 8, "block_hits is laid out as the eight-queries-per-thread k_lookup leaves it (launch_scan_tiles)");
    if (!nq) return;
    hipLaunchKernelGGL(k_lookup_windows, dim3(blocks_for(nq, KMX_WIN_TILE)), dim3(KMX_BLOCK), 0, s, ix, elem, ranks, roff, win_off, nr, nq, stride, d,
                       ctr, block_hits);
}

void launch_validate(hipStream_t s, const KmxIndexDev* ix, const uint32_t* arena, const uint8_t* qranks, const uint64_t* qoff,
                     const QueryDesc& d, uint64_t n_stitch, uint64_t n_more, uint64_t n_tiny, const uint32_t* tiny_list, uint64_t n_short,
                     uint64_t* mask_words, bool direct)
{
    if (n_tiny)
        hipLaunchKernelGGL(k_validate_tiny, dim3(blocks_for(n_tiny, KMX_BLOCK)), dim3(KMX_BLOCK), 0, s, ix, arena, qranks, qoff, d, tiny_list,
                           n_tiny, mask_words, direct && d.stitch_hits != nullptr);
    if (n_short) {
        const uint64_t swaves = (n_short + KMX_VGROUPS - 1) / KMX_VGROUPS;
        const unsigned int sblocks = (unsigned int)std::min<uint64_t>((swaves + 3) / 4, 256 * 32);
        hipLaunchKernelGGL(k_validate_short, dim3(sblocks ? sblocks : 1), dim3(KMX_BLOCK), 0, s, arena, d, n_short, mask_words);
    }
    if (!n_stitch) return;
    uint64_t waves = (n_stitch + KMX_VGROUPS - 1) / KMX_VGROUPS;
    unsigned int blocks = (unsigned int)std::min<uint64_t>((waves + 3) / 4, 256 * 32);
    const dim3 grid(blocks ? blocks : 1), block(KMX_BLOCK);
    if (n_more && !d.stitch_hits) {
        hipLaunchKernelGGL(k_validate<true>, grid, block, 0, s, ix, arena, qranks, qoff, d, n_stitch, mask_words);
        return;
    }
    hipLaunchKernelGGL(k_validate<false>, grid, block, 0, s, ix, arena, qranks, qoff, d, n_stitch, mask_words);
    if (n_more) {
        const uint64_t sw = (n_stitch + KMX_VWIDE_SCAN - 1) / KMX_VWIDE_SCAN;
        const unsigned int sblocks = (unsigned int)std::min<uint64_t>((sw + 3) / 4, 256 * 16);
        hipLaunchKernelGGL(k_validate_wide, dim3(sblocks ? sblocks : 1), dim3(KMX_VWIDE_BLOCK), 0, s, arena, d, n_stitch, mask_words);
        hipLaunchKernelGGL(k_validate_more_thread, dim3(blocks_for(n_stitch, KMX_BLOCK)), block, 0, s, ix, arena, qranks, qoff, d, n_stitch,
                           uint32_t(n_more >= KMX_VMORE_THREAD_MANY ? KMX_VMORE_THREAD_PARTS_MANY : KMX_VMORE_THREAD_PARTS), mask_words);
        hipLaunchKernelGGL(k_validate_more, grid, block, 0, s, ix, arena, qranks, qoff, d, n_stitch, mask_words);
        const uint64_t wwaves = (n_stitch + KMX_VWAVE_SCAN - 1) / KMX_VWAVE_SCAN;
        const unsigned int wblocks = (unsigned int)std::min<uint64_t>((wwaves + 3) / 4, 256 * 16);
        hipLaunchKernelGGL(k_validate_wave, dim3(wblocks ? wblocks : 1), block, 0, s, ix, arena, qranks, qoff, d, n_stitch, mask_words);
    }
}

uint64_t scan_blocks(uint64_t n) { return blocks_for(n, KMX_SCAN_TILE); }
uint64_t scan_tile() { return KMX_SCAN_TILE; }
// ... 1401 lines not shown
```

kmer_index_amd/csrc/kmx_types.h:

```cpp
#pragma once
#include <stdint.h>
#include "../../include/kmx.h"

#define KMX_MAX_LEVELS 3
#define KMX_DEFAULT_PREFIX_LEVELS 2

struct KmxSlot {
    uint64_t key;
    uint32_t off;
    uint32_t cnt;
};

struct KmxElemDev {
    uint32_t k;
    uint32_t table_kind;
    uint32_t log2cap;
    uint32_t n_ukeys;
    uint64_t n_keys;
    uint64_t arena_base;
    uint64_t npos;
    const uint32_t* offs;
    const KmxSlot* slots;
    const uint64_t* ukeys;
    const uint32_t* atab;
    uint64_t region;
    const uint32_t* dir;
    uint32_t dir_shift;
    uint32_t n_dir;
    const uint8_t* cnt8;
    uint64_t cell_base;
    uint32_t cell_shift;
    uint32_t n_levels;
    uint64_t lvl_offs_at[KMX_MAX_LEVELS];
    uint64_t lvl_base[KMX_MAX_LEVELS];
};

enum { KMX_SCHEME_NONE = 0, KMX_SCHEME_SINGLE = 1, KMX_SCHEME_MULTI = 2, KMX_SCHEME_REPLANNED = 3 };
#define KMX_PLAN_ALT_SHIFT 11
#define KMX_PLAN_NPARTS_MASK ((1u << KMX_PLAN_ALT_SHIFT) - 1u)
struct KmxPlanEntry {
    uint8_t scheme;
    uint8_t elem;
    uint16_t nparts;
};

struct KmxIndexDev {
    uint64_t n;
    uint32_t sigma;
    uint32_t n_ks;
    uint32_t kmax;
    uint32_t range;
    const uint32_t* arena;
    const uint8_t* tail;
    const KmxPlanEntry* plan;
    uint64_t arena_elems;
    unsigned long long* dbg;
    uint64_t pw[64];
    KmxElemDev elems[KMX_MAX_KS];
};

#define KMX_PSORT_IS_SMALL(runs, len) ((len) <= KMX_PSORT_CAP)
#ifndef KMX_PMERGE_MIN_AVG
#define KMX_PMERGE_MIN_AVG 8
#endif
#define KMX_PSORT_IS_MERGE(runs, len)                                                                                   \
    ((len) <= KMX_PSORT_CAP && (runs) >= 2 && (runs) <= KMX_PSORT_MAX_RUNS && !((runs) <= KMX_PMERGE_REG_RUNS && (len) <= KMX_PMERGE_REG_LEN) && \
     (len) >= KMX_PMERGE_MIN_AVG * (runs))
#ifndef KMX_PMERGE_REG_RUNS
#define KMX_PMERGE_REG_RUNS 4
#endif
#ifndef KMX_PMERGE_REG_LEN
#define KMX_PMERGE_REG_LEN 512
#endif
#define KMX_VRESOLVE 4
#define KMX_ARENA_PAD (4096 * 4 + 1024)
#define KMX_VTINY 8
#define KMX_VSHORT 16
#define KMX_PSORT_MAX_RUNS 32
#define KMX_PSORT_CAP 2048
#define KMX_PSORT_BLOCK_CAP 32768
#define KMX_PSORT_MID_CAP 8192

#define KMX_SMALL_NQ 256
#define KMX_SMALL_BLOCKS 32
struct KmxSmallArgs {
    uint16_t nq[KMX_SMALL_BLOCKS];
    uint16_t n_letters[KMX_SMALL_BLOCKS];
};
#define KMX_SMALL_IN_BYTES 8192
#define KMX_SMALL_WCAP 1024
#define KMX_SMALL_WSLOW 32
#define KMX_SMALL_SORT 4096
#define KMX_SMALL_BSLOW 8
#define KMX_SMALL_WORDS (KMX_SMALL_WSLOW * (KMX_SMALL_WCAP / 64 + 1) + KMX_SMALL_BSLOW * (KMX_SMALL_SORT / 64 + 1))
#define KMX_SMALL_POS 49152
struct KmxSmallHeader {
    uint32_t fallback;
    uint32_t nq;
    uint64_t n_hits, n_mask_words;
    uint32_t n_stitch, n_prefix, n_error, n_none;
    uint32_t pad[6];
};
struct KmxSmallLayout {
    uint32_t blocks, off_header, off_hitoff, off_csrc, off_mbase, off_ccnt, off_status, off_kinds, off_words, off_pos, bytes, pad;
};
static inline KmxSmallLayout kmx_small_layout(uint32_t blocks)
{
    KmxSmallLayout L;
    const uint32_t nq = blocks * KMX_SMALL_NQ;
    L.blocks = blocks;
    L.off_header = blocks * KMX_SMALL_IN_BYTES;
    L.off_hitoff = L.off_header + blocks * 64;
    L.off_csrc = L.off_hitoff + (nq + 2) * 8;
    L.off_mbase = L.off_csrc + nq * 8;
    L.off_ccnt = L.off_mbase + nq * 8;
    L.off_status = L.off_ccnt + nq * 4;
    L.off_kinds = L.off_status + nq;
    L.off_words = L.off_kinds + nq;
    L.off_pos = L.off_words + blocks * KMX_SMALL_WORDS * 8;
    L.bytes = L.off_pos + blocks * KMX_SMALL_POS * 4;
    L.pad = 0;
    return L;
}

enum {
    KMX_CTR_STITCH = 1,
    KMX_CTR_PREFIX = 2,
    KMX_CTR_ERROR = 3,
    KMX_CTR_MASK_WORDS = 4,
    KMX_CTR_PREFIX_ELEMS = 5,
    KMX_CTR_MAX_RUNS = 6,
    KMX_CTR_TOTAL_HITS = 7,
    KMX_CTR_NONE = 8,
    KMX_CTR_PREFIX_TOTAL = 9,
    KMX_CTR_STITCH_MORE = 10,
    KMX_CTR_PREFIX_BIG = 11,
    KMX_CTR_STITCH_TINY = 12,
    KMX_CTR_STITCH_RESOLVED = 13,
    KMX_CTR_PREFIX_MERGE = 14,
    KMX_CTR_PREFIX_MID = 15,
    KMX_CTR_PREFIX_PLAIN = 0,
    KMX_CTR_STITCH_SHORT = 16,
    KMX_CTR_LONG = 17,
    KMX_CTR_PSB_MERGE = 18,
    KMX_CTR_PSB_OTHER = 19,
    KMX_CTR_PSB_BANDS = 20,
    KMX_CTR_PSB_CUTS = 21,
    KMX_CTR_PSB_SPLITS = 22,
    KMX_CTR_COUNT = 28
};
#define KMX_LONG_PARTS 256
#define KMX_SEARCH_INTERNAL_DEFER_LONG 0x80000000u
```

kmer_index_amd/engine.py:

```python
import collections
import contextlib
import ctypes as C
import os

import numpy as np

from . import build as _build

KMX_MAX_KS = 32
KMX_MAX_DEVICES = 16
KMX_N_KERNELS = 16
TABLE_AUTO, TABLE_OPEN, TABLE_DENSE = 0, 1, 2
SEARCH_DEFAULT, SEARCH_KEEP_MASKS, SEARCH_COUNT_ONLY, SEARCH_ASYNC, SEARCH_REFERENCE_PLAN = 0, 1, 2, 4, 8
KIND_NONE, KIND_EXACT, KIND_STITCH, KIND_PREFIX = 0, 1, 2, 3
Q_OK, Q_TOO_LONG, Q_SUBK_FANOUT, Q_EMPTY_QUERY, Q_BAD_RANK, Q_TOO_SHORT = 0, 1, 2, 3, 4, 5
APPROX_MAX_SUBST = 3
APPROX_EDIT = 1
APPROX_LOCI, APPROX_BEST = 2, 4
TILE_Q_NONE, TILE_Q_PARTITION, TILE_Q_SCAN = 0, 1, 2
ALIGN_MAX_EDITS, ALIGN_MAX_READ, ALIGN_SKIPPED, ALIGN_NONE = 250, 1024, 254, 255
SCRIPT_ALL, SCRIPT_M = 1, 2
CIGAR_OPS = "MIDNSHP=X"
PAIR_FR, PAIR_RF, PAIR_FF = 0, 1, 2
PAIR_UNPLACED, PAIR_CONCORDANT, PAIR_DISCORDANT, PAIR_MATE1_ONLY, PAIR_MATE2_ONLY = 0, 1, 2, 3, 4
# ... 63 lines not shown
class MapqOptions(C.Structure):
    _fields_ = [("struct_size", C.c_uint32), ("max_edits", C.c_uint32), ("cap", C.c_uint32), ("per_edit", C.c_uint32),
                ("pair_bonus", C.c_uint32), ("flags", C.c_uint32)]


class LocateOptions(C.Structure):
    _fields_ = [("struct_size", C.c_uint32), ("flags", C.c_uint32)]


class SecondaryOptions(C.Structure):
    _fields_ = [("struct_size", C.c_uint32), ("max_secondary", C.c_uint32), ("max_delta", C.c_uint32), ("flags", C.c_uint32)]


class ClipOptions(C.Structure):
    _fields_ = [("struct_size", C.c_uint32), ("match", C.c_uint32), ("mismatch", C.c_uint32), ("gap_open", C.c_uint32),
                ("gap_extend", C.c_uint32), ("clip_penalty", C.c_uint32), ("min_score", C.c_int32), ("flags", C.c_uint32)]


class RealignOptions(C.Structure):
    _fields_ = [("struct_size", C.c_uint32), ("match", C.c_uint32), ("mismatch", C.c_uint32), ("gap_open", C.c_uint32),
                ("gap_extend", C.c_uint32), ("clip_penalty", C.c_uint32), ("min_score", C.c_int32), ("flags", C.c_uint32),
                ("scratch_bytes", C.c_uint64)]


class SupplementaryOptions(C.Structure):
    _fields_ = [("struct_size", C.c_uint32), ("max_supplementary", C.c_uint32), ("min_len", C.c_uint32), ("max_overlap", C.c_uint32),
                ("min_score", C.c_int32), ("flags", C.c_uint32)]


class PileupOptions(C.Structure):
    _fields_ = [("struct_size", C.c_uint32), ("flags", C.c_uint32), ("lo", C.c_uint64), ("hi", C.c_uint64), ("min_score", C.c_int32),
                ("min_mapq", C.c_uint32), ("mode", C.c_uint32), ("tile", C.c_uint32)]


class SitesOptions(C.Structure):
    _fields_ = [("struct_size", C.c_uint32), ("min_depth", C.c_uint32), ("min_alt", C.c_uint32), ("frac_num", C.c_uint32), ("frac_den", C.c_uint32)]


class KernelStat(C.Structure):
    _fields_ = [("name", C.c_char_p), ("launches", C.c_uint64), ("total_ms", C.c_double)]


class IndexPathInfo(C.Structure):
    _fields_ = [("struct_size", C.c_uint32), ("fill_slots", C.c_uint32), ("fill_nontemporal", C.c_uint32), ("rec64", C.c_uint32),
                ("tiny_cells", C.c_uint32), ("scan_tile", C.c_uint32), ("n_ks", C.c_uint32), ("cell_shift", C.c_uint32 * KMX_MAX_KS),
                ("windows_tile", C.c_uint32)]


class ResultPathInfo(C.Structure):
    _fields_ = [("struct_size", C.c_uint32), ("small", C.c_uint32), ("lookup_items", C.c_uint32), ("lookup_pairs", C.c_uint32),
                ("deferred_long", C.c_uint32), ("tile_q_source", C.c_uint32), ("spec_fill", C.c_uint32), ("spec_ok", C.c_uint32),
                ("fill_blocks", C.c_uint32), ("fill_tiles", C.c_uint32),
                ("prefix_plain", C.c_uint32), ("prefix_small", C.c_uint32), ("prefix_merge_small", C.c_uint32), ("prefix_mid", C.c_uint32),
                ("prefix_long", C.c_uint32), ("prefix_large_chunks", C.c_uint32), ("prefix_large_elems", C.c_uint64)]


vp, u64, u32, i32, st, P = C.c_void_p, C.c_uint64, C.c_uint32, C.c_int32, C.c_int, C.POINTER

SIGNATURES = {
    "kmx_index_build": (st, [vp, u64, u32, vp, u32, P(Options), P(vp)]),
    "kmx_index_free": (None, [vp]),
    "kmx_index_save": (st, [vp, C.c_char_p]),
    "kmx_index_load": (st, [C.c_char_p, P(Options), P(vp)]),
    "kmx_index_info": (st, [vp, P(u64), P(u32), P(u32), vp, vp, P(u64)]),
    "kmx_index_memory": (st, [vp] + [P(u64)] * 5),
    "kmx_index_arena_host": (st, [vp, P(vp), P(u64)]),
    "kmx_index_extend_query_size_range": (st, [vp, u32]),
    "kmx_index_devices": (st, [vp, P(u32), vp]),
    "kmx_index_bucket_host": (st, [vp, u32, vp, P(vp), P(u32)]),
    "kmx_index_levels": (st, [vp, vp]),
    "kmx_index_paths": (st, [vp, P(IndexPathInfo)]),
    "kmx_index_text": (st, [vp, vp, u64, P(u64)]),
    "kmx_index_set_contigs": (st, [vp, vp, u64]),
    "kmx_index_contigs": (st, [vp, P(u64), vp, u64]),
    "kmx_choose_best_k": (st, [vp, u64, u32, vp]),
    "kmx_plan": (st, [vp, u32, u32, vp, vp, vp, u64, P(u64)]),
    "kmx_plan_engine": (st, [vp, u32, u32, u32, vp]),
    "kmx_fast_pow": (u64, [u64, C.c_uint8]),
    "kmx_stats_enable": (st, [vp, C.c_int]),
    "kmx_stats_get": (st, [vp, P(KernelStat), P(u32)]),
    "kmx_stats_reset": (st, [vp]),
    "kmx_debug_words": (st, [vp, vp]),
    "kmx_last_error": (C.c_char_p, []),
    "kmx_status_string": (C.c_char_p, [C.c_int]),
    "kmx_version": (u32, []),
    "kmx_search_batch": (st, [vp, vp, vp, u64, u32, P(vp)]),
    "kmx_search_batch_device": (st, [vp, vp, vp, u64, u32, vp, P(vp)]),
    "kmx_search_windows": (st, [vp, vp, vp, u64, P(WindowOptions), P(vp)]),
    "kmx_search_windows_device": (st, [vp, vp, vp, u64, P(WindowOptions), vp, P(vp)]),
    "kmx_result_counts": (st, [vp] + [P(u64)] * 6),
    "kmx_result_view": (st, [vp] + [P(vp)] * 4),
    "kmx_result_view_device": (st, [vp] + [P(vp)] * 3),
    "kmx_result_masks": (st, [vp] + [P(vp)] * 4),
    "kmx_result_parts": (st, [vp, P(u32)]),
    "kmx_result_part_view_device": (st, [vp, u32, P(i32), P(u64), P(u64), P(vp), P(vp), P(vp)]),
    "kmx_result_gather_device": (st, [vp, i32, P(vp), P(vp), P(vp)]),
    "kmx_result_paths": (st, [vp, P(ResultPathInfo)]),
    "kmx_result_window_offsets": (st, [vp, P(vp), P(vp), P(u64)]),
    "kmx_result_free": (None, [vp]),
    "kmx_search_approx": (st, [vp, vp, vp, u64, u32, u32, P(vp)]),
    "kmx_search_approx_strands": (st, [vp, vp, vp, u64, u32, u32, vp, P(vp)]),
    "kmx_search_approx_opts": (st, [vp, vp, vp, u64, P(ApproxOptions), P(vp)]),
    "kmx_approx_counts": (st, [vp, P(u64), P(u64), P(u64), P(u32)]),
    "kmx_approx_view": (st, [vp] + [P(vp)] * 4),
    "kmx_approx_lengths": (st, [vp, P(vp)]),
    "kmx_approx_strands": (st, [vp, P(vp)]),
    "kmx_approx_found": (st, [vp, P(vp)]),
# ... 156 lines not shown
    off = np.zeros(rng + 1, np.uint32)
    n = C.c_uint64()
    _check(lib().kmx_plan(ks.ctypes.data, ks.size, rng, multi.ctypes.data, off.ctypes.data, None, 0, C.byref(n)))
    flat = np.zeros(max(n.value, 1), np.uint32)
    _check(lib().kmx_plan(ks.ctypes.data, ks.size, rng, multi.ctypes.data, off.ctypes.data, flat.ctypes.data, n.value, C.byref(n)))
    return multi.astype(bool), [flat[off[q]:off[q + 1]].tolist() for q in range(rng)]


def plan_engine(ks, sigma, rng=10000):
    ks = np.ascontiguousarray(ks, np.uint32)
    out = np.zeros(rng, np.uint32)
    _check(lib().kmx_plan_engine(ks.ctypes.data, ks.size, rng, int(sigma), out.ctypes.data))
    return out


def _view(ptr, n, dtype):
    if not ptr or n == 0:
        return np.zeros(0, dtype)
    ct = np.ctypeslib.as_ctypes_type(dtype)
    return np.ctypeslib.as_array(C.cast(ptr, C.POINTER(ct)), shape=(int(n),))


class Result:

    def __init__(self):
        self._h = C.c_void_p()
        self._index = None

    def n_parts(self):
        n = C.c_uint32()
        _check(lib().kmx_result_parts(self._h, C.byref(n)))
        return int(n.value)

    def part_device_ptrs(self, part):
        dev, qb, qe = C.c_int32(), C.c_uint64(), C.c_uint64()
        a, b, s = C.c_void_p(), C.c_void_p(), C.c_void_p()
        _check(lib().kmx_result_part_view_device(self._h, part, C.byref(dev), C.byref(qb), C.byref(qe), C.byref(a), C.byref(b), C.byref(s)))
        return int(dev.value), int(qb.value), int(qe.value), a.value, b.value, s.value

    def counts(self):
        v = [C.c_uint64() for _ in range(6)]
        _check(lib().kmx_result_counts(self._h, *[C.byref(x) for x in v]))
        return dict(zip(["nq", "n_hits", "n_exact", "n_stitch", "n_prefix", "n_error"], [int(x.value) for x in v]))

    def paths(self):
        v = ResultPathInfo()
        v.struct_size = C.sizeof(ResultPathInfo)
        _check(lib().kmx_result_paths(self._h, C.byref(v)))
        return {"small": bool(v.small), "lookup_items": int(v.lookup_items), "lookup_pairs": bool(v.lookup_pairs),
                "deferred_long": bool(v.deferred_long), "tile_q_source": int(v.tile_q_source), "spec_fill": bool(v.spec_fill),
                "spec_ok": bool(v.spec_ok), "fill_blocks": int(v.fill_blocks), "fill_tiles": int(v.fill_tiles),
                "prefix_plain": int(v.prefix_plain), "prefix_small": int(v.prefix_small), "prefix_merge_small": int(v.prefix_merge_small),
                "prefix_mid": int(v.prefix_mid), "prefix_long": int(v.prefix_long), "prefix_large_chunks": int(v.prefix_large_chunks),
                "prefix_large_elems": int(v.prefix_large_elems)}

    def host(self, copy=True):
        c = self.counts()
        a, b, s, k = C.c_void_p(), C.c_void_p(), C.c_void_p(), C.c_void_p()
        _check(lib().kmx_result_view(self._h, C.byref(a), C.byref(b), C.byref(s), C.byref(k)))
        nq = c["nq"]
        hit_off = _view(a.value, nq + 1, np.uint64)
        n_pos = int(hit_off[nq]) if b.value else 0
        out = (hit_off, _view(b.value, n_pos, np.uint32), _view(s.value, nq, np.uint8), _view(k.value, nq, np.uint8))
        return tuple(x.copy() for x in out) if copy else out

    def device_ptrs(self):
        a, b, s = C.c_void_p(), C.c_void_p(), C.c_void_p()
        _check(lib().kmx_result_view_device(self._h, C.byref(a), C.byref(b), C.byref(s)))
        return a.value, b.value, s.value

    def device_tensors(self, device):
        import torch

        class _Arr:
            def __init__(self, ptr, n, typestr):
                self.__cuda_array_interface__ = {"shape": (int(n),), "typestr": typestr, "data": (int(ptr), False), "version": 2}

        c = self.counts()
        a, b, _ = self.device_ptrs()
        t_off = torch.as_tensor(_Arr(a, c["nq"] + 1, "<i8"), device=device)
        t_pos = torch.as_tensor(_Arr(b, c["n_hits"], "<i4"), device=device) if c["n_hits"] else torch.empty(0, dtype=torch.int32, device=device)
        return t_off, t_pos

    def gather_device(self, dst_device):
        a, b, s = C.c_void_p(), C.c_void_p(), C.c_void_p()
        _check(lib().kmx_result_gather_device(self._h, int(dst_device), C.byref(a), C.byref(b), C.byref(s)))
        return a.value, b.value, s.value

    def window_offsets(self, device=False):
        a, b, n = C.c_void_p(), C.c_void_p(), C.c_uint64()
        _check(lib().kmx_result_window_offsets(self._h, C.byref(a), C.byref(b), C.byref(n)))
        win_off = _view(a.value, n.value + 1, np.uint64).copy()
        return (win_off, b.value, int(n.value)) if device else win_off

    def vote(self, band=0, min_votes=1, max_occ=0, loci=None):
        l = loci or Loci()
        o = VoteOptions(C.sizeof(VoteOptions), int(band), int(min_votes), int(max_occ), 0)
        _check(lib().kmx_windows_vote(self._h, C.byref(o), C.byref(l._h)))
        return l

    def masks(self):
        c = self.counts()
        a, b, cc, d = C.c_void_p(), C.c_void_p(), C.c_void_p(), C.c_void_p()
        _check(lib().kmx_result_masks(self._h, C.byref(a), C.byref(b), C.byref(cc), C.byref(d)))
        nq = c["nq"]
        base = _view(a.value, nq, np.uint64).copy()
        cnt = _view(cc.value, nq, np.uint32).copy()
# ... 1160 lines not shown
```

Baseline: 7094.

## Add speculative exact-only lookup kernel when previous batch was all exact

```diff
diff --git a/include/kmx.h b/include/kmx.h
--- a/include/kmx.h
+++ b/include/kmx.h
@@ -162,6 +162,8 @@
     uint32_t prefix_long;
     uint32_t prefix_large_chunks;
     uint64_t prefix_large_elems;
+    uint32_t lookup_exact;
+    uint32_t reserved0;
 } kmx_result_path_info;
 #define KMX_TILE_Q_NONE 0u
 #define KMX_TILE_Q_PARTITION 1u
diff --git a/kmer_index_amd/build.py b/kmer_index_amd/build.py
--- a/kmer_index_amd/build.py
+++ b/kmer_index_amd/build.py
@@ -6,7 +6,7 @@
 CSRC = os.path.join(HERE, "csrc")
 LIB = os.path.join(HERE, "libkmx.so")
 SOURCES = ["kmx_kernels.hip", "kmx_capi.hip", "kmx_build_sort.hip", "kmx_approx.hip", "kmx_vote.hip", "kmx_align.hip", "kmx_script.hip", "kmx_strands.hip", "kmx_pairs.hip", "kmx_rescue.hip", "kmx_tags.hip", "kmx_contigs.hip", "kmx_secondary.hip", "kmx_clip.hip", "kmx_supplementary.hip", "kmx_realign.hip", "kmx_pileup.hip", "kmx_host.cpp"]
-HEADERS = ["kmx_types.h", "kmx_host.h", "kmx_kernels.h", "kmx_approx.h", "kmx_handle.h", "kmx_vote.h", "kmx_strands.h", "kmx_clips.h", "kmx_align_core.h", "kmx_script_core.h", "kmx_runs.h", "kmx_fold_core.h", os.path.join("..", "..", "include", "kmx.h")]
+HEADERS = ["kmx_types.h", "kmx_host.h", "kmx_kernels.h", "kmx_approx.h", "kmx_handle.h", "kmx_vote.h", "kmx_strands.h", "kmx_clips.h", "kmx_align_core.h", "kmx_script_core.h", "kmx_runs.h", "kmx_fold_core.h", "kmx_exact_core.h", os.path.join("..", "..", "include", "kmx.h")]
 
 
 def _stale() -> bool:
diff --git a/kmer_index_amd/csrc/kmx_capi.hip b/kmer_index_amd/csrc/kmx_capi.hip
--- a/kmer_index_amd/csrc/kmx_capi.hip
+++ b/kmer_index_amd/csrc/kmx_capi.hip
@@ -17,6 +17,7 @@
 
 #include "kmx_approx.h"
 #include "kmx_host.h"
+#include "kmx_exact_core.h"
 #include "kmx_kernels.h"
 #include "kmx_vote.h"
 
@@ -185,6 +186,7 @@
     KmxIndexDev h_header{};
     kmx::FillVariant fill_variant{12, true};
     bool rec32 = true;
+    bool exact_front = true;
     bool tiny_cells = false;
     bool broken = false;
     std::vector<uint32_t> host_arena;
@@ -248,7 +250,8 @@
     bool last_had_stitch = false;
     bool last_had_long = false;
     bool last_had_pairs = false;
-    struct PathRec { uint32_t small = 0, items = 0, pairs = 0, defer_long = 0, tile_q_source = 0, spec_fill = 0, spec_ok = 0, fill_blocks = 0, fill_tiles = 0;
+    bool last_all_exact = false;
+    struct PathRec { uint32_t small = 0, items = 0, pairs = 0, defer_long = 0, exact = 0, tile_q_source = 0, spec_fill = 0, spec_ok = 0, fill_blocks = 0, fill_tiles = 0;
                      uint32_t p_plain = 0, p_small = 0, p_merge = 0, p_mid = 0, p_long = 0, p_chunks = 0; uint64_t p_elems = 0; };
     PathRec path;
     std::shared_ptr<ResultPool> pool;
@@ -408,6 +411,18 @@
     return shift;
 }
 static inline uint64_t up32_elems(uint64_t v) { return (v + 31) & ~uint64_t(31); }
+
+static void derive_header_fields(KmxIndexDev& h)
+{
+    uint32_t j = 0;
+    while (j < 63 && h.pw[j + 1] <= KMX_SUBK_FANOUT_LIMIT) ++j;
+    h.max_fan_exp = j;
+    bool small = true;
+    for (uint32_t e = 0; e < h.n_ks; ++e) small = small && kmx_exact::small_keys_ok(h.sigma, h.elems[e].n_keys);
+    h.small_keys = small ? 1u : 0u;
+}
+
+constexpr uint64_t kExactCnt8Max = uint64_t(4) << 20;
 
 static hipError_t publish_headers(kmx_index* ix)
 {
@@ -580,6 +595,7 @@
             }
             if (ce != hipSuccess) { fail(ce == hipErrorOutOfMemory ? KMX_ERR_OUT_OF_MEMORY : KMX_ERR_HIP, std::string("cells: ") + hipGetErrorString(ce)); return bail(KMX_ERR_HIP); }
             el.cnt8 = static_cast<const uint8_t*>(p);
+            if (im.n_keys > kExactCnt8Max) ix->exact_front = false;
             if (im.npos <= 4 * im.n_keys) ix->tiny_cells = true;
             ix->bytes_cells += ((im.n_keys << cell_shift[i]) * 4) + im.n_keys;
             el.cell_base = cell_base[i];
@@ -592,6 +608,7 @@
         base += im.region;
         im = kmx::ElemImage();
     }
+    derive_header_fields(h);
     ix->host_dirs.reset(new kmx_index::HostDir[n_ks]);
     ix->tail.assign(tail_kmax, tail_kmax + kmax);
     if ((st = upload(ix, tail_kmax, kmax, &h.tail)) != KMX_OK) return bail(st);
@@ -621,7 +638,7 @@
     ix->device = device;
     ix->n = src->n; ix->sigma = src->sigma; ix->range = src->range;
     ix->ks = src->ks; ix->table_kinds = src->table_kinds; ix->elem_sizes = src->elem_sizes; ix->tail = src->tail;
-    ix->fill_variant = src->fill_variant; ix->rec32 = src->rec32; ix->tiny_cells = src->tiny_cells;
+    ix->fill_variant = src->fill_variant; ix->rec32 = src->rec32; ix->tiny_cells = src->tiny_cells; ix->exact_front = src->exact_front;
     ix->bytes_positions = src->bytes_positions; ix->bytes_aligned = src->bytes_aligned; ix->bytes_cells = src->bytes_cells; ix->bytes_levels = src->bytes_levels;
     auto bail = [&](kmx_status s) { std::string keep = g_err; kmx_index_free(ix); g_err = keep; return s; };
     hipError_t e = hipSetDevice(device);
@@ -1416,6 +1433,7 @@
     v.fill_blocks = r->path.fill_blocks; v.fill_tiles = r->path.fill_tiles;
     v.prefix_plain = r->path.p_plain; v.prefix_small = r->path.p_small; v.prefix_merge_small = r->path.p_merge; v.prefix_mid = r->path.p_mid;
     v.prefix_long = r->path.p_long; v.prefix_large_chunks = r->path.p_chunks; v.prefix_large_elems = r->path.p_elems;
+    v.lookup_exact = r->path.exact;
     v.struct_size = std::min<uint32_t>(out->struct_size, uint32_t(sizeof v));
     memcpy(out, &v, v.struct_size);
     return KMX_OK;
@@ -1508,6 +1526,12 @@
 }
 
 using LookupStep = std::function<int(const kmx::QueryDesc&, unsigned long long*, const KmxIndexDev*)>;
+static kmx_status enqueue_front(kmx_index* ix, kmx_result* r, const LookupStep& lookup);
+static int forced_lookup_items()
+{
+    static const int force_items = getenv("KMX_LOOKUP_ITEMS") ? atoi(getenv("KMX_LOOKUP_ITEMS")) : 0;
+    return force_items;
+}
 static kmx_status search_device_run(kmx_index* ix, kmx_result* r, const uint8_t* qr, const uint64_t* qo, uint64_t nq, uint32_t flags, hipStream_t s,
                                     const LookupStep& lookup)
 {
@@ -1536,12 +1560,30 @@
         r->ctr_phase = 0;
         r->ctr_clean = true;
     }
-    const kmx::QueryDesc d = r->query_desc();
     if (!r->ctr_clean) {
         HIP_TRY(hipMemsetAsync(r->ctr.p, 0, 2 * kCtrBytes, s));
         r->ctr_clean = true;
     }
     r->ctr_phase ^= 1u;
+    r->ctx = SearchCtx{ix, qr, qo, s, 0, 0, false, false};
+    KMX_TRY(enqueue_front(ix, r, lookup));
+    r->ctx.pending = true;
+    if (flags & KMX_SEARCH_ASYNC) {
+        if (!r->done) HIP_TRY(hipEventCreateWithFlags(&r->done, hipEventDisableTiming));
+        HIP_TRY(hipEventRecord(r->done, s));
+        r->pool = ix->pool;
+        std::lock_guard<std::mutex> lock(ix->pool->mu);
+        ix->pool->pending.push_back(r);
+        return KMX_OK;
+    }
+    return search_finish(r);
+}
+
+static kmx_status enqueue_front(kmx_index* ix, kmx_result* r, const LookupStep& lookup)
+{
+    const uint32_t flags = r->flags;
+    hipStream_t s = r->ctx.s;
+    const kmx::QueryDesc d = r->query_desc();
     auto* ctr = r->ctr_block(r->ctr_phase);
     auto* ctr_next = r->ctr_block(r->ctr_phase ^ 1u);
     const KmxIndexDev* dix = header_for(ix, flags);
@@ -1561,16 +1603,26 @@
         });
     r->path.spec_fill = spec_fill;
     if (!published) HIP_TRY(hipMemcpyAsync(r->h_ctr, ctr, kCtrBytes, hipMemcpyDeviceToHost, s));
-    r->ctx = SearchCtx{ix, qr, qo, s, tile_cap, spec_tiles, spec_fill, true};
-    if (flags & KMX_SEARCH_ASYNC) {
-        if (!r->done) HIP_TRY(hipEventCreateWithFlags(&r->done, hipEventDisableTiming));
-        HIP_TRY(hipEventRecord(r->done, s));
-        r->pool = ix->pool;
-        std::lock_guard<std::mutex> lock(ix->pool->mu);
-        ix->pool->pending.push_back(r);
-        return KMX_OK;
-    }
-    return search_finish(r);
+    r->ctx.tile_cap = tile_cap; r->ctx.spec_tiles = spec_tiles; r->ctx.spec_fill = spec_fill;
+    return KMX_OK;
+}
+
+static int lookup_general(kmx_index* ix, kmx_result* r, const kmx::QueryDesc& d, unsigned long long* ctr, const KmxIndexDev* dix)
+{
+    const uint8_t* qr = r->ctx.qr; const uint64_t* qo = r->ctx.qo;
+    const uint32_t flags = r->flags;
+    hipStream_t s = r->ctx.s;
+    const int force_items = forced_lookup_items();
+    const bool pairs = force_items ? force_items == -4 : r->last_had_pairs;
+    const int items = force_items ? (force_items == 8 ? 8 : 4) : (!pairs && ix->tiny_cells) ? 8 : 4;
+    const bool defer_long = r->last_had_long;
+    const uint32_t lflags = (flags & ~KMX_SEARCH_INTERNAL_DEFER_LONG) | (defer_long ? KMX_SEARCH_INTERNAL_DEFER_LONG : 0u);
+    r->path.items = uint32_t(items); r->path.pairs = pairs; r->path.defer_long = defer_long; r->path.exact = 0;
+    timed(ix, K_LOOKUP, s, [&] {
+        kmx::launch_lookup(s, items, pairs, dix, qr, qo, r->nq, d, ctr, r->bsum.as<uint64_t>(), lflags);
+        if (defer_long) kmx::launch_lookup_long(s, dix, qr, qo, r->nq, d, ctr, flags);
+    });
+    return items;
 }
 
 kmx_status kmx_search_batch_device(const kmx_index* cix, const void* d_qranks, const void* d_qoff, uint64_t nq,
@@ -1587,15 +1639,11 @@
     kmx_result* r = *inout;
     r->windows = false;
     return search_device_run(ix, r, qr, qo, nq, flags, s, [&](const kmx::QueryDesc& d, unsigned long long* ctr, const KmxIndexDev* dix) {
-        static const int force_items = getenv("KMX_LOOKUP_ITEMS") ? atoi(getenv("KMX_LOOKUP_ITEMS")) : 0;
-        const bool pairs = force_items ? force_items == -4 : r->last_had_pairs;
-        const int items = force_items ? (force_items == 8 ? 8 : 4) : (!pairs && ix->tiny_cells) ? 8 : 4;
-        const bool defer_long = r->last_had_long;
-        const uint32_t lflags = (flags & ~KMX_SEARCH_INTERNAL_DEFER_LONG) | (defer_long ? KMX_SEARCH_INTERNAL_DEFER_LONG : 0u);
-        r->path.items = uint32_t(items); r->path.pairs = pairs; r->path.defer_long = defer_long;
+        if (!r->last_all_exact || !ix->exact_front || forced_lookup_items()) return lookup_general(ix, r, d, ctr, dix);
+        const int items = ix->tiny_cells ? 8 : 4;
+        r->path.items = uint32_t(items); r->path.pairs = 0; r->path.defer_long = 0; r->path.exact = 1;
         timed(ix, K_LOOKUP, s, [&] {
-            kmx::launch_lookup(s, items, pairs, dix, qr, qo, nq, d, ctr, r->bsum.as<uint64_t>(), lflags);
-            if (defer_long) kmx::launch_lookup_long(s, dix, qr, qo, nq, d, ctr, flags);
+            kmx::launch_lookup_exact(s, items, ix->h_header.small_keys != 0, dix, qr, qo, nq, d, ctr, r->bsum.as<uint64_t>());
         });
         return items;
     });
@@ -1792,6 +1840,7 @@
     r->last_had_stitch = c.stitch_pending != 0;
     r->last_had_long = h[KMX_CTR_LONG] != 0;
     r->last_had_pairs = r->n_stitch != 0;
+    r->last_all_exact = !r->windows && r->n_stitch == 0 && r->n_prefix == 0 && h[KMX_CTR_LONG] == 0 && h[KMX_CTR_NOT_EXACT] == 0;
     r->path.p_plain = uint32_t(c.prefix_plain); r->path.p_merge = uint32_t(c.prefix_merge); r->path.p_mid = uint32_t(c.prefix_mid);
     r->path.p_small = uint32_t(c.prefix_small - std::min(c.prefix_small, c.prefix_merge));
     r->path.p_long = uint32_t(c.prefix_big - std::min(c.prefix_big, c.prefix_mid));
@@ -1962,6 +2011,14 @@
     r->ctx.pending = false;
     KMX_TRY(wait_counters(r));
     kmx_index* ix = r->ctx.ix;
+    if (r->path.exact && r->h_ctr[KMX_CTR_NOT_EXACT] != 0) {
+        r->last_all_exact = false;
+        HIP_TRY(hipMemsetAsync(r->ctr.p, 0, 2 * kCtrBytes, r->ctx.s));
+        r->ctr_clean = true;
+        r->path = kmx_result::PathRec{};
+        KMX_TRY(enqueue_front(ix, r, [&](const kmx::QueryDesc& d, unsigned long long* ctr, const KmxIndexDev* dix) { return lookup_general(ix, r, d, ctr, dix); }));
+        HIP_TRY(hipStreamSynchronize(r->ctx.s));
+    }
     const kmx::FillVariant fv = kmx::effective_fill_variant(ix->fill_variant, ix->rec32);
     Finish f{r, ix, r->ctx.s, r->query_desc(), r->ctr_block(r->ctr_phase), header_for(ix, r->flags), fv, kmx::fill_tile(fv), read_counts(r)};
     if (f.c.stitch_pending) KMX_TRY(f.validate_stitch());
@@ -2035,7 +2092,7 @@
     if (n_letters) memcpy(r->small_in.as<unsigned char>() + (nq + 1) * 8, qranks + l0, n_letters);
     r->host_valid = r->host_masks_valid = r->small_valid = r->quiesced = true;
     r->windows = false; r->path = kmx_result::PathRec{}; r->path.small = 1;
-    r->last_had_stitch = r->last_had_pairs = r->last_had_long = false;
+    r->last_had_stitch = r->last_had_pairs = r->last_had_long = r->last_all_exact = false;
     r->pool = ix->pool;
     *served = true;
     return KMX_OK;
diff --git a/kmer_index_amd/csrc/kmx_exact_core.h b/kmer_index_amd/csrc/kmx_exact_core.h
--- /dev/null
+++ b/kmer_index_amd/csrc/kmx_exact_core.h
@@ -0,0 +1,74 @@
+#pragma once
+#include <stdint.h>
+
+#if defined(__HIPCC__)
+#include <hip/hip_runtime.h>
+#define KMX_EXACT_HD __host__ __device__ __forceinline__
+#else
+#define KMX_EXACT_HD inline
+#endif
+
+namespace kmx_exact {
+
+constexpr uint32_t kBlock = 256;
+constexpr uint32_t kPerThread = 4;
+constexpr uint32_t kStage = 12288;
+constexpr uint32_t kChunk = 16;
+constexpr uint32_t kMaxLen = 64;
+
+constexpr uint32_t threads_of(uint32_t items) { return kBlock * items / kPerThread; }
+
+struct Tile { uint64_t base, end; };
+KMX_EXACT_HD Tile tile_of(uint64_t block, uint32_t items, uint64_t nq)
+{
+    Tile t;
+    t.base = block * uint64_t(kBlock) * items;
+    t.end = t.base + uint64_t(kBlock) * items < nq ? t.base + uint64_t(kBlock) * items : nq;
+    return t;
+}
+KMX_EXACT_HD uint64_t first_query(const Tile& t, uint32_t thread) { return t.base + uint64_t(thread) * kPerThread; }
+KMX_EXACT_HD uint32_t live_queries(const Tile& t, uint64_t q0)
+{
+    return q0 >= t.end ? 0u : t.end - q0 < kPerThread ? uint32_t(t.end - q0) : kPerThread;
+}
+KMX_EXACT_HD uint64_t offset_index(const Tile& t, uint64_t q0, uint32_t i) { return q0 + i < t.end ? q0 + i : t.end; }
+
+KMX_EXACT_HD bool piece_staged(uint64_t lo, uint64_t hi) { return hi - lo <= kStage; }
+KMX_EXACT_HD uint32_t chunk_bytes(uint32_t i, uint32_t len) { return i >= len ? 0u : len - i < kChunk ? len - i : kChunk; }
+KMX_EXACT_HD bool inside_piece(uint64_t b, uint64_t m, uint64_t lo, uint64_t hi) { return b >= lo && b <= hi && m <= hi - b; }
+
+template <bool SMALL, typename Fetch>
+KMX_EXACT_HD bool exact_hash(Fetch fetch, uint64_t pos, uint32_t k, uint32_t sigma, uint64_t* h)
+{
+    uint32_t top = 0;
+    if (SMALL) {
+        uint32_t acc = 0;
+        for (uint32_t t = 0; t < k; ++t) {
+            const uint32_t c = fetch(pos + t);
+            top = c > top ? c : top;
+#if defined(__HIP_DEVICE_COMPILE__)
+            acc = __umul24(acc, sigma) + c;
+#else
+            acc = (acc & 0xFFFFFFu) * (sigma & 0xFFFFFFu) + c;
+#endif
+        }
+        *h = acc;
+    } else {
+        uint64_t acc = 0;
+        for (uint32_t t = 0; t < k; ++t) {
+            const uint32_t c = fetch(pos + t);
+            top = c > top ? c : top;
+            acc = acc * sigma + c;
+        }
+        *h = acc;
+    }
+    return top < sigma;
+}
+KMX_EXACT_HD bool small_keys_ok(uint32_t sigma, uint64_t n_keys)
+{
+    return sigma < (1u << 24) && n_keys <= (uint64_t(1) << 32) && n_keys / sigma <= (uint64_t(1) << 24);
+}
+
+KMX_EXACT_HD bool vector_stores(uint32_t live, uint32_t served) { return live == kPerThread && served == kPerThread; }
+
+}
diff --git a/kmer_index_amd/csrc/kmx_kernels.h b/kmer_index_amd/csrc/kmx_kernels.h
--- a/kmer_index_amd/csrc/kmx_kernels.h
+++ b/kmer_index_amd/csrc/kmx_kernels.h
@@ -26,6 +26,8 @@
                    uint64_t nq, const QueryDesc& d, unsigned long long* ctr, uint64_t* block_hits, uint32_t flags);
 void launch_lookup_long(hipStream_t s, const KmxIndexDev* ix, const uint8_t* qranks, const uint64_t* qoff, uint64_t nq, const QueryDesc& d,
                         unsigned long long* ctr, uint32_t flags);
+void launch_lookup_exact(hipStream_t s, int items, bool small_keys, const KmxIndexDev* ix, const uint8_t* qranks, const uint64_t* qoff, uint64_t nq, const QueryDesc& d,
+                         unsigned long long* ctr, uint64_t* block_hits);
 uint64_t windows_tile();
 int windows_items();
 void launch_window_counts(hipStream_t s, const uint64_t* roff, uint64_t nr, uint32_t w, uint32_t stride, uint32_t* cnt);
diff --git a/kmer_index_amd/csrc/kmx_kernels.hip b/kmer_index_amd/csrc/kmx_kernels.hip
--- a/kmer_index_amd/csrc/kmx_kernels.hip
+++ b/kmer_index_amd/csrc/kmx_kernels.hip
@@ -5,6 +5,7 @@
 #include <atomic>
 #include <type_traits>
 
+#include "kmx_exact_core.h"
 #include "kmx_kernels.h"
 
 #define KMX_BLOCK 256
@@ -434,8 +435,7 @@
     unsigned int max_runs;
     unsigned int base_stitch, base_stitch_tiny, base_stitch_short, base_prefix, base_prefix_big;
     unsigned long long base_words;
-    unsigned int max_fan_exp;
-    unsigned int small_keys;
+    unsigned int n_not_exact;
 };
 
 template <bool SMALL>
@@ -534,15 +534,7 @@
         bc.n_stitch = bc.n_stitch_tiny = bc.n_stitch_short = bc.n_resolved = bc.n_prefix = bc.n_prefix_big = bc.n_prefix_merge = bc.n_prefix_mid = bc.n_prefix_plain = bc.n_error = bc.n_none = bc.n_more = 0;
         bc.words = bc.pelems = bc.hits = 0;
         bc.max_runs = 0;
-        unsigned int j = 0;
-        while (j < 63 && ix->pw[j + 1] <= KMX_SUBK_FANOUT_LIMIT) ++j;
-        bc.max_fan_exp = j;
-        unsigned int small = ix->sigma < (1u << 24) ? 1u : 0u;
-        for (uint32_t e = 0; e < ix->n_ks; ++e) {
-            const uint64_t nk = ix->elems[e].n_keys;
-            if (nk > (uint64_t(1) << 32) || nk / ix->sigma > (uint64_t(1) << 24)) small = 0;
-        }
-        bc.small_keys = small;
+        bc.n_not_exact = 0;
     }
     {
         const uint32_t n_words = ix->n_ks * uint32_t(sizeof(KmxElemDev) / 8);
@@ -560,7 +552,8 @@
     bool done[ITEMS];
     uint64_t my_hits = 0;
     const uint32_t sigma = ix->sigma, range = ix->range;
-    const bool small_keys = __builtin_amdgcn_readfirstlane(int(bc.small_keys)) != 0;
+    const bool small_keys = ix->small_keys != 0;
+    const uint32_t max_fan_exp = ix->max_fan_exp;
     const uint8_t* __restrict__ dummy = reinterpret_cast<const uint8_t*>(ix);
 
     unsigned int my_resolved = 0, my_err = 0, my_none = 0;
@@ -651,13 +644,14 @@
             const uint32_t m = qm[it], scheme = praw[it] & 0xFF, e = (praw[it] >> 8) & 0xFF;
             const uint32_t kb = elems_s[e].k;
             const bool live = q < nq && m > 0 && m < range;
+            if (q < nq && !(live && scheme == KMX_SCHEME_SINGLE && kb == m)) atomicAdd(&bc.n_not_exact, 1u);
             const bool one = live && scheme == KMX_SCHEME_SINGLE && kb == m && m <= 16 && qranks + qb[it] + 16 <= qend;
             bool t = false;
             uint32_t ea = e, off = 0;
             if (PAIRS && live && !one && m < KMX_PLAN_LDS) {
                 if (scheme == KMX_SCHEME_SINGLE) {
                     const uint32_t rest = m < 2 * kb ? m - kb : 0u;
-                    t = m > kb && m <= 2 * kb && kb <= 16 && (rest == 0 || kb - rest <= bc.max_fan_exp);
+                    t = m > kb && m <= 2 * kb && kb <= 16 && (rest == 0 || kb - rest <= max_fan_exp);
                     off = m - kb;
                 } else if (scheme == KMX_SCHEME_MULTI && ((praw[it] >> 16) & KMX_PLAN_NPARTS_MASK) == 2 && m > kb) {
                     const uint32_t p2 = plan_s[m - kb];
@@ -857,6 +851,7 @@
         if (bc.n_resolved) atomicAdd(&ctr[KMX_CTR_STITCH_RESOLVED], (unsigned long long)bc.n_resolved);
         if (bc.n_error) atomicAdd(&ctr[KMX_CTR_ERROR], (unsigned long long)bc.n_error);
         if (bc.n_none) atomicAdd(&ctr[KMX_CTR_NONE], (unsigned long long)bc.n_none);
+        if (bc.n_not_exact) atomicAdd(&ctr[KMX_CTR_NOT_EXACT], (unsigned long long)bc.n_not_exact);
     }
     __syncthreads();
 #pragma unroll
@@ -1123,6 +1118,173 @@
         block_hits[blockIdx.x] = s_hits;
         if (s_err) atomicAdd(&ctr[KMX_CTR_ERROR], (unsigned long long)s_err);
         if (s_none) atomicAdd(&ctr[KMX_CTR_NONE], (unsigned long long)s_none);
+    }
+}
+
+typedef unsigned long long u64x2_a8 __attribute__((ext_vector_type(2), aligned(8)));
+
+template <int TILE_ITEMS, bool SMALL>
+__global__ __launch_bounds__(kmx_exact::threads_of(TILE_ITEMS), 8) void k_lookup_exact(const KmxIndexDev* __restrict__ ix, const uint8_t* __restrict__ qranks,
+                                                               const uint64_t* __restrict__ qoff, uint64_t nq, QueryDesc d,
+                                                               unsigned long long* __restrict__ ctr, uint64_t* __restrict__ block_hits)
+{
+    constexpr int ITEMS = kmx_exact::kPerThread;
+    constexpr uint32_t THREADS = kmx_exact::threads_of(TILE_ITEMS);
+    static_assert(KMX_BLOCK == kmx_exact::kBlock && THREADS >= kmx_exact::kMaxLen, "one planner entry per thread of the first wave");
+    static_assert(ITEMS == 4, "kind and status leave as one 4-byte store, cnt as one 16-byte store");
+    __shared__ KmxElemDev elems_s[KMX_MAX_KS];
+    __shared__ uint8_t s_elem[kmx_exact::kMaxLen];
+    __shared__ unsigned int s_err, s_none, s_unserved;
+    __shared__ unsigned long long s_hits;
+    __shared__ __attribute__((aligned(16))) uint8_t s_let[kmx_exact::kStage];
+    const kmx_exact::Tile tile = kmx_exact::tile_of(blockIdx.x, TILE_ITEMS, nq);
+    const uint64_t q0 = kmx_exact::first_query(tile, threadIdx.x);
+    const uint32_t live = kmx_exact::live_queries(tile, q0);
+
+    const uint64_t lo = qoff[tile.base], hi = qoff[tile.end];
+    uint64_t o[ITEMS + 1];
+    if (live == ITEMS) {
+#pragma unroll
+        for (int i = 0; i < ITEMS; i += 2) {
+            const u64x2_a8 v = *reinterpret_cast<const u64x2_a8*>(qoff + q0 + i);
+            o[i] = v.x; o[i + 1] = v.y;
+        }
+        o[ITEMS] = qoff[q0 + ITEMS];
+    } else {
+#pragma unroll
+        for (int i = 0; i <= ITEMS; ++i) o[i] = qoff[kmx_exact::offset_index(tile, q0, uint32_t(i))];
+    }
+    uint32_t praw = 0;
+    if (threadIdx.x > 0 && threadIdx.x < kmx_exact::kMaxLen && threadIdx.x < ix->range)
+        praw = plan_effective(((const KMX_GLOBAL uint32_t*)ix->plan)[threadIdx.x]);
+    {
+        const uint32_t n_words = ix->n_ks * uint32_t(sizeof(KmxElemDev) / 8);
+        const uint64_t* __restrict__ srcw = reinterpret_cast<const uint64_t*>(ix->elems);
+        uint64_t* dstw = reinterpret_cast<uint64_t*>(elems_s);
+        for (uint32_t i = threadIdx.x; i < n_words; i += THREADS) dstw[i] = srcw[i];
+    }
+    if (threadIdx.x == 0) {
+        s_err = s_none = s_unserved = 0;
+        s_hits = 0;
+    }
+    __syncthreads();
+    if (threadIdx.x < kmx_exact::kMaxLen) {
+        const uint32_t e = (praw >> 8) & 0xFF;
+        s_elem[threadIdx.x] = ((praw & 0xFF) == KMX_SCHEME_SINGLE && e < ix->n_ks && elems_s[e].k == threadIdx.x) ? uint8_t(e) : uint8_t(0xFF);
+    }
+    const bool staged = kmx_exact::piece_staged(lo, hi);
+    if (staged) {
+        const uint32_t len = uint32_t(hi - lo);
+        for (uint32_t i = threadIdx.x * kmx_exact::kChunk; i < len; i += THREADS * kmx_exact::kChunk) {
+            if (kmx_exact::chunk_bytes(i, len) == kmx_exact::kChunk) {
+                *reinterpret_cast<u32x4*>(s_let + i) = *reinterpret_cast<const u32x4_a1*>(qranks + lo + i);
+            } else {
+                for (uint32_t j = i; j < len; ++j) s_let[j] = qranks[lo + j];
+            }
+        }
+    }
+    __syncthreads();
+
+    const uint32_t sigma = ix->sigma;
+    auto element_of = [&](uint64_t b, uint64_t m) -> uint32_t {
+        const uint32_t e = m < kmx_exact::kMaxLen ? s_elem[uint32_t(m)] : 0xFFu;
+        return (kmx_exact::inside_piece(b, m, lo, hi) && b - lo <= 0xFFFFFFFFull) ? e : 0xFFu;
+    };
+    uint32_t rel[ITEMS], el[ITEMS];
+    unsigned int served = 0;
+#pragma unroll
+    for (int i = 0; i < ITEMS; ++i) {
+        el[i] = uint32_t(i) < live ? element_of(o[i], o[i + 1] - o[i]) : 0xFFu;
+        rel[i] = uint32_t(o[i] - lo);
+        served += el[i] != 0xFFu;
+    }
+    unsigned int n_unserved = live - served, my_err = 0, my_none = 0;
+    uint64_t my_hits = 0;
+    const uint8_t* __restrict__ piece = qranks + lo;
+    if (kmx_exact::vector_stores(live, served)) {
+        typename std::conditional<SMALL, uint32_t, uint64_t>::type hs[ITEMS];
+        uint32_t bad = 0;
+        auto hashes = [&](auto fetch) {
+#pragma unroll
+            for (int i = 0; i < ITEMS; ++i) {
+                uint64_t h = 0;
+                if (!kmx_exact::exact_hash<SMALL>(fetch, rel[i], elems_s[el[i]].k, sigma, &h)) bad |= 1u << i;
+                hs[i] = decltype(hs[i] + 0)(h);
+            }
+        };
+        if (staged) hashes([&](uint64_t p) -> uint32_t { return s_let[uint32_t(p)]; });
+        else hashes([&](uint64_t p) -> uint32_t { return piece[p]; });
+        const char* dummy = reinterpret_cast<const char*>(ix);
+        u32x4_a1 pr[ITEMS];
+#pragma unroll
+        for (int i = 0; i < ITEMS; ++i)
+            pr[i] = *(const KMX_GLOBAL u32x4_a1*)(!((bad >> i) & 1u) ? probe_first_addr(&elems_s[el[i]], hs[i]) : dummy);
+        uint32_t kw = 0, sw = 0;
+        uint64_t src_even = 0;
+        u32x4 cv;
+#pragma unroll
+        for (int i = 0; i < ITEMS; ++i) {
+            const bool is_bad = (bad >> i) & 1u;
+            Run r{0, 0};
+            if (!is_bad) r = probe_finish(&elems_s[el[i]], hs[i], pr[i]);
+            my_err += is_bad;
+            my_none += !is_bad && !r.cnt;
+            my_hits += r.cnt;
+            kw |= uint32_t(r.cnt ? KMX_KIND_EXACT : KMX_KIND_NONE) << (8 * i);
+            sw |= uint32_t(is_bad ? KMX_Q_BAD_RANK : KMX_Q_OK) << (8 * i);
+            if (i & 1) {
+                u64x2 v;
+                v.x = src_even; v.y = r.src;
+                *reinterpret_cast<u64x2*>(d.src + q0 + i - 1) = v;
+            } else src_even = r.src;
+            if ((i & 3) == 0) cv.x = r.cnt; else if ((i & 3) == 1) cv.y = r.cnt; else if ((i & 3) == 2) cv.z = r.cnt;
+            else {
+                cv.w = r.cnt;
+                *reinterpret_cast<u32x4*>(d.cnt + q0 + i - 3) = cv;
+            }
+        }
+        *reinterpret_cast<uint32_t*>(d.kind + q0) = kw;
+        *reinterpret_cast<uint32_t*>(d.status + q0) = sw;
+    } else {
+#pragma unroll 1
+        for (uint32_t i = 0; i < live; ++i) {
+            const uint64_t q = q0 + i, b = qoff[q];
+            const uint32_t e = element_of(b, qoff[q + 1] - b);
+            Run r{~uint64_t(0), 0};
+            if (e != 0xFFu) {
+                uint64_t h = 0;
+                const uint32_t k = elems_s[e].k;
+                const bool ok = staged ? kmx_exact::exact_hash<SMALL>([&](uint64_t p) -> uint32_t { return s_let[uint32_t(p)]; }, b - lo, k, sigma, &h)
+                                       : kmx_exact::exact_hash<SMALL>([&](uint64_t p) -> uint32_t { return piece[p]; }, b - lo, k, sigma, &h);
+                r = ok ? probe(&elems_s[e], h) : Run{0, 0};
+                my_err += !ok;
+                my_none += ok && !r.cnt;
+                my_hits += r.cnt;
+                d.kind[q] = r.cnt ? uint8_t(KMX_KIND_EXACT) : uint8_t(KMX_KIND_NONE);
+                d.status[q] = ok ? uint8_t(KMX_Q_OK) : uint8_t(KMX_Q_BAD_RANK);
+            }
+            d.src[q] = r.src;
+            d.cnt[q] = r.cnt;
+        }
+    }
+    for (int off = 32; off > 0; off >>= 1) {
+        my_hits += __shfl_xor(my_hits, off);
+        my_err += __shfl_xor(my_err, off);
+        my_none += __shfl_xor(my_none, off);
+        n_unserved += __shfl_xor(n_unserved, off);
+    }
+    if (lane_id() == 0) {
+        if (my_hits) atomicAdd(&s_hits, (unsigned long long)my_hits);
+        if (my_err) atomicAdd(&s_err, my_err);
+        if (my_none) atomicAdd(&s_none, my_none);
+        if (n_unserved) atomicAdd(&s_unserved, n_unserved);
+    }
+    __syncthreads();
+    if (threadIdx.x == 0) {
+        block_hits[blockIdx.x] = s_hits;
+        if (s_err) atomicAdd(&ctr[KMX_CTR_ERROR], (unsigned long long)s_err);
+        if (s_none) atomicAdd(&ctr[KMX_CTR_NONE], (unsigned long long)s_none);
+        if (s_unserved) atomicAdd(&ctr[KMX_CTR_NOT_EXACT], (unsigned long long)s_unserved);
     }
 }
 
@@ -3401,6 +3563,14 @@
     else hipLaunchKernelGGL((k_lookup<4, false>), grid, block, 0, s, ix, qranks, qoff, nq, d, ctr, block_hits, flags);
 }
 
+void launch_lookup_exact(hipStream_t s, int items, bool small_keys, const KmxIndexDev* ix, const uint8_t* qranks, const uint64_t* qoff, uint64_t nq, const QueryDesc& d,
+                         unsigned long long* ctr, uint64_t* block_hits)
+{
+    if (nq == 0) return;
+    const dim3 grid(unsigned(lookup_blocks(nq, items == 8 ? 8 : 4))), block(kmx_exact::threads_of(items == 8 ? 8 : 4));
+    auto* kernel = items == 8 ? (small_keys ? k_lookup_exact<8, true> : k_lookup_exact<8, false>) : (small_keys ? k_lookup_exact<4, true> : k_lookup_exact<4, false>);
+    hipLaunchKernelGGL(kernel, grid, block, 0, s, ix, qranks, qoff, nq, d, ctr, block_hits);
+}
 uint64_t windows_tile() { return KMX_WIN_TILE; }
 int windows_items() { return KMX_WIN_ITEMS; }
 
diff --git a/kmer_index_amd/csrc/kmx_types.h b/kmer_index_amd/csrc/kmx_types.h
--- a/kmer_index_amd/csrc/kmx_types.h
+++ b/kmer_index_amd/csrc/kmx_types.h
@@ -55,6 +55,8 @@
     const KmxPlanEntry* plan;
     uint64_t arena_elems;
     unsigned long long* dbg;
+    uint32_t max_fan_exp;
+    uint32_t small_keys;
     uint64_t pw[64];
     KmxElemDev elems[KMX_MAX_KS];
 };
@@ -147,6 +149,7 @@
     KMX_CTR_PSB_BANDS = 20,
     KMX_CTR_PSB_CUTS = 21,
     KMX_CTR_PSB_SPLITS = 22,
+    KMX_CTR_NOT_EXACT = 26,
     KMX_CTR_COUNT = 28
 };
 #define KMX_LONG_PARTS 256
diff --git a/kmer_index_amd/engine.py b/kmer_index_amd/engine.py
--- a/kmer_index_amd/engine.py
+++ b/kmer_index_amd/engine.py
@@ -139,7 +139,8 @@
                 ("deferred_long", C.c_uint32), ("tile_q_source", C.c_uint32), ("spec_fill", C.c_uint32), ("spec_ok", C.c_uint32),
                 ("fill_blocks", C.c_uint32), ("fill_tiles", C.c_uint32),
                 ("prefix_plain", C.c_uint32), ("prefix_small", C.c_uint32), ("prefix_merge_small", C.c_uint32), ("prefix_mid", C.c_uint32),
-                ("prefix_long", C.c_uint32), ("prefix_large_chunks", C.c_uint32), ("prefix_large_elems", C.c_uint64)]
+                ("prefix_long", C.c_uint32), ("prefix_large_chunks", C.c_uint32), ("prefix_large_elems", C.c_uint64),
+                ("lookup_exact", C.c_uint32), ("reserved0", C.c_uint32)]
 
 
 vp, u64, u32, i32, st, P = C.c_void_p, C.c_uint64, C.c_uint32, C.c_int32, C.c_int, C.POINTER
@@ -402,7 +403,7 @@
                 "spec_ok": bool(v.spec_ok), "fill_blocks": int(v.fill_blocks), "fill_tiles": int(v.fill_tiles),
                 "prefix_plain": int(v.prefix_plain), "prefix_small": int(v.prefix_small), "prefix_merge_small": int(v.prefix_merge_small),
                 "prefix_mid": int(v.prefix_mid), "prefix_long": int(v.prefix_long), "prefix_large_chunks": int(v.prefix_large_chunks),
-                "prefix_large_elems": int(v.prefix_large_elems)}
+                "prefix_large_elems": int(v.prefix_large_elems), "lookup_exact": bool(v.lookup_exact)}
 
     def host(self, copy=True):
         c = self.counts()
```

Result: no change. 7069 (-0.3%).
